# vocdoni/zk-franchise-proof-circuit

Measured on AMD Instinct MI355X. Metric: zkCensus proofs/sec (nLevels=160), higher is better.
Workload: dtype u256 (8 x u32 Montgomery, BN254 Fr/Fq)

## Files before the change

### include/zkcensus.h

```cpp
#ifndef ZKCENSUS_H
#define ZKCENSUS_H
#include <stddef.h>
#include <stdint.h>
#ifdef __cplusplus
extern "C" {
#endif

typedef struct zkc_ctx zkc_ctx;
typedef struct zkc_zkey zkc_zkey;

enum {
    ZKC_OK = 0,
    ZKC_ERR_GENERIC = 1,
    ZKC_ERR_SHORT_BUFFER = 2,
    ZKC_ERR_INVALID_WITNESS_LENGTH = 3,
    ZKC_ERR_BAD_ARG = 4,
    ZKC_ERR_FORMAT = 5,
    ZKC_ERR_HIP = 6,
    ZKC_ERR_WITNESS = 7
};
enum {
    ZKC_W_OK = 0, ZKC_W_ERR_WEIGHT = 1 , ZKC_W_ERR_SIK_ROOT = 2 ,
    ZKC_W_ERR_CENSUS_ROOT = 3 , ZKC_W_ERR_NULLIFIER = 4 , ZKC_W_ERR_LAST_SIBLING = 5 ,
    ZKC_W_ERR_INPUT_RANGE = 6 ,
// ... 64 lines not shown
                             uint8_t proof[256], uint8_t* publics, zkc_done_fn done, void* user);
int zkc_service_stats(zkc_service* svc, uint64_t out[8]);
int zkc_service_timing(zkc_service* svc, uint64_t out[8]);
int zkc_service_memory(zkc_service* svc, uint64_t out[8]);

int groth16_prover(const void* zkey_buffer, unsigned long zkey_size, const void* wtns_buffer, unsigned long wtns_size,
                   char* proof_buffer, unsigned long* proof_size, char* public_buffer, unsigned long* public_size,
                   char* error_msg, unsigned long error_msg_maxsize);

int groth16_fullprove(const void* zkey_buffer, unsigned long zkey_size, const void* wasm_buffer, unsigned long wasm_size, const char* inputs_json, unsigned long inputs_size,
                      char* proof_buffer, unsigned long* proof_size, char* public_buffer, unsigned long* public_size,
                      char* error_msg, unsigned long error_msg_maxsize);

int zkc_verify(const char* vkey_json, const char* public_json, const char* proof_json);
int zkc_verify_bin(const uint8_t* vk, int nPublic, const uint8_t* pub, const uint8_t* proof);

int zkc_pairing_bin(const uint8_t g1[64], const uint8_t g2[128], uint8_t out[384]);

int zkc_verify_batch(zkc_ctx* ctx, const uint8_t* vk, int nPublic, const uint8_t* pubs, const uint8_t* proofs, int N, const uint8_t* seed32);
const char* zkc_verify_last_error(void);

int zkc_proof_to_json(const uint8_t proof[256], const uint8_t* pub, int nPublic, char* proof_buf, unsigned long* proof_size,
                      char* public_buf, unsigned long* public_size);
int zkc_proof_from_json(const char* proof_json, const char* public_json, uint8_t proof[256], uint8_t* pub, int* nPublic);
int zkc_vkey_from_json(const char* vkey_json, uint8_t* vk, unsigned long* vk_size, int* nPublic);
int zkc_wtns_parse(const void* wtns_bytes, unsigned long size, const uint8_t** payload, uint32_t* nWitness);
unsigned long zkc_wtns_write(const void* payload, uint32_t nWitness, void* out, unsigned long out_size);

typedef struct zkc_msm zkc_msm;
int zkc_ntt_dev(zkc_ctx* ctx, const void* d_src, void* d_dst, int logn, int nvec, int inverse);
int zkc_g1_mul_batch_dev(zkc_ctx* ctx, const uint8_t base_std[64], const void* d_scalars, uint32_t n, void* d_out);
int zkc_msm_g1_load_dev(zkc_ctx* ctx, const void* d_bases_std, uint32_t n, zkc_msm** out);
int zkc_msm_g1_dev(zkc_msm* m, const void* d_scalars, uint8_t out[64]);
void zkc_msm_g1_free(zkc_msm* m);

int zkc_debug_stage(zkc_zkey* zk, const void* d_wtns, int stage, void* host_out);
unsigned long long zkc_debug_early_retries(void);
int zkc_msm_debug(zkc_zkey* zk, int which, const void* d_scalars, uint32_t count, void* host_out);
int zkc_debug_pairing_dev(zkc_ctx* ctx, const uint8_t* g1, const uint8_t* g2, const uint8_t* weights, int N, uint8_t product_out[384], uint8_t* folded_out,
                          int32_t* member_out, int* bad_out, const uint32_t* nodes, size_t count, uint8_t* node_out);

int zkc_poseidon_batch(zkc_ctx* ctx, int n_inputs, const void* inputs, size_t B, void* out);
int zkc_smt_build(zkc_ctx* ctx, const void* keys, const void* values, size_t n, int nLevels, uint8_t root[32], void* siblings, int32_t* depths);
int zkc_census_inputs(zkc_ctx* ctx, size_t n, int nLevels, const uint8_t election_id[64], const void* address, const void* password, const void* signature,
                      const void* available_weight, const void* vote_weight, const void* vote_hash, void* inputs_out, void* d_inputs_out, uint8_t* roots_out);

typedef struct zkc_tree zkc_tree;
enum {
    ZKC_TREE_OK = 0,
    ZKC_TREE_KEY_EXISTS = 1,
    ZKC_TREE_KEY_ABSENT = 2,
    ZKC_TREE_COLLISION = 3,
    ZKC_TREE_NOT_BELOW_R = 4,
    ZKC_TREE_NOT_IN_CENSUS = 5,
    ZKC_TREE_NOT_IN_SIK = 6,
    ZKC_TREE_SIK_MISMATCH = 7
};
int  zkc_tree_create(zkc_ctx* ctx, int nLevels, zkc_tree** out);
void zkc_tree_free(zkc_tree* tree);
int  zkc_tree_add(zkc_tree* tree, const void* keys, const void* values, size_t n, int32_t* status);
int  zkc_tree_update(zkc_tree* tree, const void* keys, const void* values, size_t n, int32_t* status);
int  zkc_tree_root(zkc_tree* tree, uint8_t root[32]);
int  zkc_tree_size(zkc_tree* tree, size_t* leaves);
int  zkc_tree_get(zkc_tree* tree, const void* keys, size_t n, void* values_out, int32_t* exists);
int  zkc_tree_gen_proof(zkc_tree* tree, const void* keys, size_t n, uint8_t root[32], void* siblings, int32_t* depths, int32_t* exists);
int  zkc_tree_census_inputs(zkc_tree* census, zkc_tree* sik, size_t n, const uint8_t election_id[64], const void* address, const void* password, const void* signature,
                            const void* vote_weight, const void* vote_hash, void* inputs_out, void* d_inputs_out, uint8_t roots_out[64], int32_t* status);
int  zkc_tree_stats(zkc_tree* tree, double ms[2]);

enum {
    ZKC_SMT_VALID = 0,
    ZKC_SMT_ROOT_MISMATCH = 1,
    ZKC_SMT_NOT_BELOW_R = 2,
    ZKC_SMT_LAST_SIBLING = 3,
    ZKC_SMT_KEY_PRESENT = 4,
    ZKC_SMT_OFF_PATH = 5
};
int zkc_smt_check_proofs(zkc_ctx* ctx, int nLevels, size_t n, const void* keys, const void* values, const void* siblings, const void* roots, int per_proof_roots,
                         int32_t* status);
int zkc_smt_check_stats(zkc_ctx* ctx, double ms[3]);

int zkc_profile_enable(zkc_ctx* ctx, uint32_t mask);
int zkc_profile_read(zkc_ctx* ctx, int category, double* total_ms, uint64_t* launches, uint64_t* alg_bytes);

int zkc_setup_from_r1cs(const char* r1cs_path, uint64_t seed, const char* zkey_path, const char* vkey_json_path,
                        char* err, size_t errlen);

#ifdef __cplusplus
}
#endif
#include "zkcensus_delete.h"
#include "zkcensus_snapshot.h"
#include "zkcensus_verify_each.h"
#include "zkcensus_setup.h"
#include "zkcensus_r1cs.h"
#include "zkcensus_phase2.h"
#endif
```

### zk-franchise-proof-circuit_amd/_native.py

```python
import ctypes
import os

_HERE = os.path.dirname(os.path.abspath(__file__))
LIB_PATH = os.environ.get('ZKCENSUS_LIB') or os.path.join(_HERE, 'libzkcensus.so')
_lib = None


class ZkcError(RuntimeError):
    def __init__(self, code, msg):
        super().__init__('libzkcensus error %d: %s' % (code, msg))
        self.code = code


def load():
    global _lib
    if _lib is not None:
        return _lib
    if not os.path.exists(LIB_PATH):
        raise ImportError('libzkcensus.so is not built (run `python -c "import __graft_entry__ as g; g.build()"`); '
                          'there is no CPU fallback for the product path')
    try:
        import torch
    except ImportError:
        pass
    L = ctypes.CDLL(LIB_PATH)
    vp, i32p = ctypes.c_void_p, ctypes.POINTER(ctypes.c_int32)
    L.zkc_ctx_create.argtypes = [ctypes.c_int, ctypes.POINTER(vp)]
    L.zkc_ctx_destroy.argtypes = [vp]
    L.zkc_last_error.argtypes = [vp]; L.zkc_last_error.restype = ctypes.c_char_p
    L.zkc_ctx_stream.argtypes = [vp]; L.zkc_ctx_stream.restype = vp
    L.zkc_witness.argtypes = [vp, ctypes.c_int, vp, ctypes.c_int, vp, i32p]
    L.zkc_witness_dev.argtypes = [vp, ctypes.c_int, vp, ctypes.c_int, vp, vp]
    u8p, u32p = ctypes.c_char_p, ctypes.POINTER(ctypes.c_uint32)
    L.zkc_zkey_load.argtypes = [vp, ctypes.c_char_p, ctypes.c_size_t, ctypes.POINTER(vp)]
    L.zkc_zkey_free.argtypes = [vp]; L.zkc_zkey_free.restype = None
    L.zkc_zkey_info.argtypes = [vp, u32p, u32p, u32p]
    L.zkc_zkey_pass_info.argtypes = [vp, ctypes.POINTER(ctypes.c_int), ctypes.POINTER(ctypes.c_int)]
    L.zkc_witness_status_text.argtypes = [ctypes.c_int, ctypes.c_int32]; L.zkc_witness_status_text.restype = ctypes.c_char_p
    L.zkc_prove.argtypes = [vp, ctypes.c_char_p, ctypes.c_uint32, u8p, u8p, ctypes.c_char_p, ctypes.c_char_p]
    L.zkc_prove_dev.argtypes = [vp, vp, ctypes.c_uint32, u8p, u8p, ctypes.c_char_p, ctypes.c_char_p]
    L.zkc_prove_batch_dev.argtypes = [vp, vp, ctypes.c_uint32, ctypes.c_int, ctypes.c_char_p, ctypes.c_char_p, ctypes.c_char_p]
    L.zkc_fullprove_batch_dev.argtypes = [vp, vp, ctypes.c_int, vp, vp, ctypes.c_char_p, ctypes.c_char_p, ctypes.c_char_p]
    L.zkc_debug_stage.argtypes = [vp, vp, ctypes.c_int, ctypes.c_char_p]
    L.zkc_debug_early_retries.argtypes = []; L.zkc_debug_early_retries.restype = ctypes.c_ulonglong
    L.zkc_msm_debug.argtypes = [vp, ctypes.c_int, vp, ctypes.c_uint32, ctypes.c_char_p]
    L.zkc_debug_pairing_dev.argtypes = [vp, ctypes.c_char_p, ctypes.c_char_p, ctypes.c_char_p, ctypes.c_int, ctypes.c_char_p, ctypes.c_char_p, i32p, ctypes.POINTER(ctypes.c_int),
                                        ctypes.POINTER(ctypes.c_uint32), ctypes.c_size_t, ctypes.c_char_p]
    ulp = ctypes.POINTER(ctypes.c_ulong)
    L.groth16_prover.argtypes = [ctypes.c_char_p, ctypes.c_ulong, ctypes.c_char_p, ctypes.c_ulong, ctypes.c_char_p, ulp, ctypes.c_char_p, ulp, ctypes.c_char_p, ctypes.c_ulong]
    L.zkc_verify.argtypes = [ctypes.c_char_p, ctypes.c_char_p, ctypes.c_char_p]
    L.zkc_verify_bin.argtypes = [ctypes.c_char_p, ctypes.c_int, ctypes.c_char_p, ctypes.c_char_p]
    L.zkc_verify_batch.argtypes = [vp, ctypes.c_char_p, ctypes.c_int, ctypes.c_char_p, ctypes.c_char_p, ctypes.c_int, ctypes.c_char_p]
    L.zkc_verify_batch_each.argtypes = [vp, ctypes.c_char_p, ctypes.c_int, ctypes.c_char_p, ctypes.c_char_p, ctypes.c_int, ctypes.c_char_p, i32p]
    L.zkc_verify_each_stats.argtypes = [vp, ctypes.POINTER(ctypes.c_uint64)]
    L.zkc_verify_last_error.restype = ctypes.c_char_p
    L.zkc_proof_to_json.argtypes = [ctypes.c_char_p, ctypes.c_char_p, ctypes.c_int, ctypes.c_char_p, ulp, ctypes.c_char_p, ulp]
    L.zkc_proof_from_json.argtypes = [ctypes.c_char_p, ctypes.c_char_p, ctypes.c_char_p, ctypes.c_char_p, ctypes.POINTER(ctypes.c_int)]
    L.zkc_vkey_from_json.argtypes = [ctypes.c_char_p, ctypes.c_char_p, ulp, ctypes.POINTER(ctypes.c_int)]
    L.zkc_wtns_parse.argtypes = [ctypes.c_char_p, ctypes.c_ulong, ctypes.POINTER(ctypes.c_void_p), ctypes.POINTER(ctypes.c_uint32)]
    L.zkc_wtns_write.argtypes = [ctypes.c_char_p, ctypes.c_uint32, ctypes.c_char_p, ctypes.c_ulong]; L.zkc_wtns_write.restype = ctypes.c_ulong
    L.zkc_poseidon_batch.argtypes = [vp, ctypes.c_int, ctypes.c_char_p, ctypes.c_size_t, ctypes.c_char_p]
    L.zkc_smt_build.argtypes = [vp, ctypes.c_char_p, ctypes.c_char_p, ctypes.c_size_t, ctypes.c_int, ctypes.c_char_p, ctypes.c_char_p, i32p]
    L.zkc_census_inputs.argtypes = [vp, ctypes.c_size_t, ctypes.c_int, ctypes.c_char_p, ctypes.c_char_p, ctypes.c_char_p, ctypes.c_char_p, ctypes.c_char_p, ctypes.c_char_p, ctypes.c_char_p, vp, vp, ctypes.c_char_p]
    sz = ctypes.c_size_t
    L.zkc_tree_create.argtypes = [vp, ctypes.c_int, ctypes.POINTER(vp)]
    L.zkc_tree_free.argtypes = [vp]; L.zkc_tree_free.restype = None
    L.zkc_tree_add.argtypes = [vp, ctypes.c_char_p, ctypes.c_char_p, sz, i32p]
    L.zkc_tree_update.argtypes = [vp, ctypes.c_char_p, ctypes.c_char_p, sz, i32p]
    L.zkc_tree_delete.argtypes = [vp, ctypes.c_char_p, sz, i32p]
    L.zkc_tree_refs.argtypes = [vp, ctypes.POINTER(sz)]
    L.zkc_tree_snapshot.argtypes = [vp, ctypes.POINTER(vp)]
    L.zkc_tree_snapshot_count.argtypes = [vp, ctypes.POINTER(sz)]
    L.zkc_tree_gen_absence_proof.argtypes = [vp, ctypes.c_char_p, sz, ctypes.c_char_p, vp, i32p, vp, vp, i32p, i32p]
    L.zkc_tree_root.argtypes = [vp, ctypes.c_char_p]
    L.zkc_tree_size.argtypes = [vp, ctypes.POINTER(sz)]
    L.zkc_tree_get.argtypes = [vp, ctypes.c_char_p, sz, vp, i32p]
    L.zkc_tree_gen_proof.argtypes = [vp, ctypes.c_char_p, sz, ctypes.c_char_p, vp, i32p, i32p]
    L.zkc_tree_census_inputs.argtypes = [vp, vp, sz, ctypes.c_char_p, ctypes.c_char_p, ctypes.c_char_p, ctypes.c_char_p, ctypes.c_char_p, ctypes.c_char_p, vp, vp, ctypes.c_char_p, i32p]
    L.zkc_tree_stats.argtypes = [vp, ctypes.POINTER(ctypes.c_double)]
    L.zkc_smt_check_proofs.argtypes = [vp, ctypes.c_int, sz, ctypes.c_char_p, ctypes.c_char_p, ctypes.c_char_p, ctypes.c_char_p, ctypes.c_int, i32p]
    L.zkc_smt_check_absence.argtypes = [vp, ctypes.c_int, sz, ctypes.c_char_p, ctypes.c_char_p, ctypes.c_char_p, i32p, ctypes.c_char_p, ctypes.c_char_p, ctypes.c_int, i32p]
    L.zkc_smt_check_stats.argtypes = [vp, ctypes.POINTER(ctypes.c_double)]
    L.zkc_profile_enable.argtypes = [vp, ctypes.c_uint32]
    L.zkc_ntt_dev.argtypes = [vp, vp, vp, ctypes.c_int, ctypes.c_int, ctypes.c_int]
    L.zkc_g1_mul_batch_dev.argtypes = [vp, ctypes.c_char_p, vp, ctypes.c_uint32, vp]
    L.zkc_msm_g1_load_dev.argtypes = [vp, vp, ctypes.c_uint32, ctypes.POINTER(vp)]
    L.zkc_msm_g1_dev.argtypes = [vp, vp, ctypes.c_char_p]
    L.zkc_msm_g1_free.argtypes = [vp]; L.zkc_msm_g1_free.restype = None
    L.zkc_profile_read.argtypes = [vp, ctypes.c_int, ctypes.POINTER(ctypes.c_double), ctypes.POINTER(ctypes.c_uint64), ctypes.POINTER(ctypes.c_uint64)]
    L.zkc_setup_from_r1cs.argtypes = [ctypes.c_char_p, ctypes.c_uint64, ctypes.c_char_p, ctypes.c_char_p, ctypes.c_char_p, ctypes.c_size_t]
    L.zkc_setup_from_r1cs_dev.argtypes = [vp, ctypes.c_char_p, ctypes.c_uint64, ctypes.c_char_p, ctypes.c_char_p, ctypes.c_char_p, ctypes.c_size_t]
    L.zkc_setup_stats.argtypes = [ctypes.POINTER(ctypes.c_double)]
    L.zkc_g1_fixed_mul_dev.argtypes = [vp, ctypes.c_char_p, vp, ctypes.c_uint32, vp]
    L.zkc_g2_fixed_mul_dev.argtypes = [vp, ctypes.c_char_p, vp, ctypes.c_uint32, vp]
    L.zkc_fixed_mul_window.argtypes = []
    L.zkc_circuit_nlevels_from_wasm.argtypes = [ctypes.c_char_p, ctypes.c_size_t, ctypes.c_char_p]
    L.zkc_sha256.argtypes = [ctypes.c_char_p, ctypes.c_size_t, ctypes.c_char_p]; L.zkc_sha256.restype = None
    L.zkc_zkey_sha256.argtypes = [vp, ctypes.c_char_p]
    L.zkc_zkey_fingerprint.argtypes = [ctypes.c_char_p, ctypes.c_size_t, ctypes.c_char_p]
    L.zkc_random_scalars.argtypes = [ctypes.c_char_p, ctypes.c_size_t]; L.zkc_random_scalars.restype = None
    L.zkc_pairing_bin.argtypes = [ctypes.c_char_p, ctypes.c_char_p, ctypes.c_char_p]
    L.zkc_pool_create.argtypes = [ctypes.POINTER(ctypes.c_int), ctypes.c_int, ctypes.POINTER(vp)]
    L.zkc_pool_destroy.argtypes = [vp]; L.zkc_pool_destroy.restype = None
    L.zkc_pool_size.argtypes = [vp]
    L.zkc_pool_ctx.argtypes = [vp, ctypes.c_int]; L.zkc_pool_ctx.restype = vp
    L.zkc_pool_zkey.argtypes = [vp, ctypes.c_int]; L.zkc_pool_zkey.restype = vp
    L.zkc_pool_last_error.argtypes = [vp]; L.zkc_pool_last_error.restype = ctypes.c_char_p
    L.zkc_pool_zkey_load.argtypes = [vp, ctypes.c_char_p, ctypes.c_size_t]
    L.zkc_pool_fullprove_batch.argtypes = [vp, ctypes.c_char_p, ctypes.c_int, ctypes.c_char_p, ctypes.c_char_p, ctypes.c_char_p, i32p]
    L.zkc_batch_begin.argtypes = [vp, ctypes.c_int, vp, ctypes.c_int, vp, vp, ctypes.c_char_p]
    L.zkc_batch_finish.argtypes = [vp, ctypes.c_int, ctypes.c_char_p, ctypes.c_char_p]
    L.zkc_service_create.argtypes = [ctypes.POINTER(ctypes.c_int), ctypes.c_int, ctypes.POINTER(vp)]
    L.zkc_service_destroy.argtypes = [vp]; L.zkc_service_destroy.restype = None
    L.zkc_service_default.argtypes = []; L.zkc_service_default.restype = vp
    L.zkc_service_last_error.restype = ctypes.c_char_p
    L.zkc_service_fullprove.argtypes = [vp, ctypes.c_char_p, ctypes.c_size_t, ctypes.c_int, ctypes.c_char_p, ctypes.c_char_p, ctypes.c_char_p, ctypes.c_char_p, i32p, ctypes.c_char_p, ctypes.c_size_t]
    L.zkc_service_prove.argtypes = [vp, ctypes.c_char_p, ctypes.c_size_t, ctypes.c_char_p, ctypes.c_uint32, ctypes.c_char_p, ctypes.c_char_p, ctypes.c_char_p, ctypes.c_char_p, ctypes.c_size_t]
    L.zkc_service_stats.argtypes = [vp, ctypes.POINTER(ctypes.c_uint64)]
    L.zkc_service_timing.argtypes = [vp, ctypes.POINTER(ctypes.c_uint64)]
    L.zkc_inputs_from_json.argtypes = [ctypes.c_char_p, ctypes.c_size_t, ctypes.c_int, ctypes.c_char_p, ctypes.c_char_p, ctypes.c_size_t]
    L.zkc_service_fullprove_json.argtypes = [vp, ctypes.c_char_p, ctypes.c_size_t, ctypes.c_char_p, ctypes.c_size_t, ctypes.c_char_p, ctypes.c_size_t, ctypes.c_char_p, ctypes.c_char_p, ctypes.c_char_p, i32p, ctypes.c_char_p, ctypes.c_size_t]
    L.groth16_fullprove.argtypes = [ctypes.c_char_p, ctypes.c_ulong, ctypes.c_char_p, ctypes.c_ulong, ctypes.c_char_p, ctypes.c_ulong, ctypes.c_char_p, ulp, ctypes.c_char_p, ulp, ctypes.c_char_p, ctypes.c_ulong]
    L.zkc_service_memory.argtypes = [vp, ctypes.POINTER(ctypes.c_uint64)]
    L.zkc_service_submit_fullprove.argtypes = [vp, ctypes.c_char_p, ctypes.c_size_t, ctypes.c_int, ctypes.c_char_p, ctypes.c_char_p, ctypes.c_char_p, ctypes.c_char_p, vp, vp]
    u32p_, i64p = u32p, ctypes.POINTER(ctypes.c_int64)
    L.zkc_r1cs_header_info.argtypes = [ctypes.c_char_p, sz, u32p_, u32p_, u32p_]
    L.zkc_r1cs_load.argtypes = [vp, ctypes.c_char_p, sz, ctypes.POINTER(vp)]
    L.zkc_r1cs_free.argtypes = [vp]; L.zkc_r1cs_free.restype = None
    L.zkc_r1cs_info.argtypes = [vp, u32p_, u32p_, u32p_]
    L.zkc_r1cs_check.argtypes = [vp, ctypes.c_char_p, ctypes.c_uint32, ctypes.c_int, i64p, u32p_]
    L.zkc_r1cs_check_dev.argtypes = [vp, vp, ctypes.c_uint32, ctypes.c_int, i64p, u32p_]
    L.zkc_r1cs_check_stats.argtypes = [vp, ctypes.POINTER(ctypes.c_double)]
    u64p = ctypes.POINTER(ctypes.c_uint64)
    szp = ctypes.POINTER(sz)
    L.zkc_g1_scale_dev.argtypes = [vp, vp, ctypes.c_uint32, ctypes.c_char_p, ctypes.c_int, vp]
    L.zkc_blake2b512.argtypes = [ctypes.c_char_p, sz, ctypes.c_char_p]; L.zkc_blake2b512.restype = None
    L.zkc_zkey_contributions.argtypes = [ctypes.c_char_p, sz, ctypes.c_char_p, u32p, ctypes.c_char_p, szp, ctypes.c_char_p, sz]
    L.zkc_zkey_contribute.argtypes = [vp, ctypes.c_char_p, sz, ctypes.c_char_p, ctypes.c_char_p, ctypes.c_char_p, szp, ctypes.c_char_p]
    L.zkc_zkey_verify_contributions.argtypes = [vp, ctypes.c_char_p, sz, ctypes.c_char_p, sz, ctypes.c_char_p, u32p, ctypes.c_char_p, sz]
    L.zkc_phase2_stats.argtypes = [ctypes.POINTER(ctypes.c_double)]
    L.zkc_debug_phase2_challenge_g2.argtypes = [ctypes.c_char_p, ctypes.c_char_p]
    L.zkc_debug_phase2_host_scale.argtypes = [ctypes.c_char_p, ctypes.c_uint32, ctypes.c_char_p, ctypes.c_int, ctypes.c_char_p, ctypes.POINTER(ctypes.c_double)]
    _lib = L
    return L


def declared_symbols(header='zkcensus.h'):
    import re
    hdr = open(os.path.join(_HERE, '..', 'include', header)).read()
    hdr = re.sub(r'/\*.*?\*/', '', hdr, flags=re.S)
    return sorted(set(re.findall(r'\b((?:zkc|groth16)_[a-z0-9_]+)\s*\(', hdr)))
```

### zk-franchise-proof-circuit_amd/csrc/zkc_api.hip

```cpp
#include "zkc_internal.h"
#include "zkc_f29.h"
#include "zkc_kernels.h"
#include <array>
#include <cstring>
#include <ctime>
#include <map>
#include <mutex>
#include "../../include/zkc_poseidon_constants.inc"

using namespace zkc;

static constexpr int ZKC_WITNESS_WAVE_MAX_B = 128, ZKC_WITNESS_WAVE_MAX_B_ALONE = 1024;

static thread_local std::string g_create_err;

int zkc_fail(zkc_ctx* ctx, int code, const std::string& msg) {
    if (ctx) ctx->err = msg; else g_create_err = msg;
    return code;
}
hipError_t zkc_wait_event(hipEvent_t ev, unsigned spin_us) {
    if (sw::on<sw::ZKC_SPIN_WAIT>()) return hipEventSynchronize(ev);
    timespec t0; if (spin_us) clock_gettime(CLOCK_MONOTONIC, &t0);
    for (int i = 0;; i++) {
        const hipError_t e = hipEventQuery(ev);
        if (e != hipErrorNotReady) return e;
        if (i < 48) continue;
        if (spin_us) { timespec t; clock_gettime(CLOCK_MONOTONIC, &t); if ((t.tv_sec - t0.tv_sec) * 1000000ll + (t.tv_nsec - t0.tv_nsec) / 1000 < (long long)spin_us) continue; spin_us = 0; }
        timespec ts{0, 50000}; nanosleep(&ts, nullptr);
    }
}
hipError_t zkc_wait_stream(hipStream_t st, hipEvent_t scratch_ev) {
    const hipError_t e = hipEventRecord(scratch_ev, st);
    return e != hipSuccess ? e : zkc_wait_event(scratch_ev);
}
int zkc_ensure(zkc_ctx* ctx, void** p, size_t* cur, size_t need) {
    if (*cur >= need) return ZKC_OK;
    if (*p) { ZKC_HIP_CHECK(ctx, hipFree(*p)); *p = nullptr; *cur = 0; }
    ZKC_HIP_CHECK(ctx, hipMalloc(p, need));
    *cur = need;
    return ZKC_OK;
}

void zkc_verify_ws_trim(zkc_ctx* ctx, size_t keep_bytes) {
    size_t total = 0; for (size_t b : ctx->vws_sz) total += b;
    if (total <= keep_bytes && keep_bytes) return;
    for (int i = 0; i < zkc_ctx::VWS_N; i++) { if (ctx->vws[i]) (void)hipFree(ctx->vws[i]); ctx->vws[i] = nullptr; ctx->vws_sz[i] = 0; }
}

static hipEvent_t prof_event(zkc_ctx* ctx) {
    if (!ctx->prof.free_events.empty()) { hipEvent_t e = ctx->prof.free_events.back(); ctx->prof.free_events.pop_back(); return e; }
    hipEvent_t e = nullptr; (void)hipEventCreate(&e); return e;
}
zkc_prof_scope::zkc_prof_scope(zkc_ctx* c, int category, uint64_t alg_bytes, hipStream_t stream) : ctx(c), cat(category), st(stream ? stream : (c ? c->stream : nullptr)) {
    on = c && ((c->prof.mask >> category) & 1u);
    if (!on) return;
    a = prof_event(c); b = prof_event(c);
    c->prof.bytes[cat] += alg_bytes; c->prof.launches[cat] += 1;
    (void)hipEventRecord(a, st);
}
zkc_prof_scope::~zkc_prof_scope() {
    if (!on) return;
    (void)hipEventRecord(b, st);
    ctx->prof.pending.push_back({a, b, cat});
}
extern "C" int zkc_profile_enable(zkc_ctx* ctx, uint32_t mask) {
    if (!ctx) return ZKC_ERR_BAD_ARG;
    ZKC_LOCK(ctx);
    ZKC_HIP_CHECK(ctx, hipSetDevice(ctx->device));
    (void)hipStreamSynchronize(ctx->stream);
    for (auto& r : ctx->prof.pending) { ctx->prof.free_events.push_back(r.a); ctx->prof.free_events.push_back(r.b); }
    ctx->prof.pending.clear();
    for (int i = 0; i < ZKC_PROF_NCAT; i++) { ctx->prof.ms[i] = 0; ctx->prof.launches[i] = 0; ctx->prof.bytes[i] = 0; }
    if (!ctx->d_prof_entries && hipMalloc((void**)&ctx->d_prof_entries, 8) != hipSuccess) ctx->d_prof_entries = nullptr;
    if (ctx->d_prof_entries) (void)hipMemset(ctx->d_prof_entries, 0, 8);
    ctx->prof.mask = mask;
    return ZKC_OK;
}
extern "C" int zkc_profile_read(zkc_ctx* ctx, int cat, double* total_ms, uint64_t* launches, uint64_t* alg_bytes) {
    if (!ctx || cat < 0 || cat >= ZKC_PROF_NCAT) return ZKC_ERR_BAD_ARG;
    ZKC_LOCK(ctx);
    ZKC_HIP_CHECK(ctx, hipSetDevice(ctx->device));
    ZKC_HIP_CHECK(ctx, hipStreamSynchronize(ctx->stream)); ZKC_HIP_CHECK(ctx, hipStreamSynchronize(ctx->stream2)); ZKC_HIP_CHECK(ctx, hipStreamSynchronize(ctx->fin_stream));
    for (auto& r : ctx->prof.pending) {
        float ms = 0; (void)hipEventElapsedTime(&ms, r.a, r.b); ctx->prof.ms[r.cat] += ms;
        ctx->prof.free_events.push_back(r.a); ctx->prof.free_events.push_back(r.b);
    }
    ctx->prof.pending.clear();
    if (cat == ZKC_PROF_MSM_G1_STREAMED && ctx->d_prof_entries) {
        unsigned long long v = 0; (void)hipMemcpyAsync(&v, ctx->d_prof_entries, 8, hipMemcpyDeviceToHost, ctx->stream); (void)hipStreamSynchronize(ctx->stream); ctx->prof.launches[cat] = v;
    }
    if (total_ms) *total_ms = ctx->prof.ms[cat]; if (launches) *launches = ctx->prof.launches[cat]; if (alg_bytes) *alg_bytes = ctx->prof.bytes[cat];
    return ZKC_OK;
}

extern "C" int zkc_poseidon_batch(zkc_ctx* ctx, int n_inputs, const void* inputs, size_t B, void* out) {
    if (!ctx || !inputs || !out || n_inputs < 2 || n_inputs > 4 || B == 0) return zkc_fail(ctx, ZKC_ERR_BAD_ARG, "zkc_poseidon_batch: bad argument");
    ZKC_LOCK(ctx);
    ZKC_HIP_CHECK(ctx, hipSetDevice(ctx->device));
    int rc;
    if ((rc = zkc_ensure(ctx, &ctx->d_scratch_in, &ctx->scratch_in_sz, B * n_inputs * 32))) return rc;
    if ((rc = zkc_ensure(ctx, &ctx->d_scratch_out, &ctx->scratch_out_sz, B * 32))) return rc;
    ZKC_HIP_CHECK(ctx, hipMemcpyAsync(ctx->d_scratch_in, inputs, B * n_inputs * 32, hipMemcpyHostToDevice, ctx->stream));
    hipLaunchKernelGGL(zkc_poseidon_batch_kernel, dim3((unsigned)((B + 63) / 64)), dim3(64), 0, ctx->stream, ctx->ptab, (const uint32_t*)ctx->d_scratch_in,
                       (uint32_t*)ctx->d_scratch_out, n_inputs, B);
    ZKC_HIP_CHECK(ctx, hipGetLastError());
    ZKC_HIP_CHECK(ctx, hipMemcpyAsync(out, ctx->d_scratch_out, B * 32, hipMemcpyDeviceToHost, ctx->stream));
    ZKC_HIP_CHECK(ctx, hipStreamSynchronize(ctx->stream));
    return ZKC_OK;
}

__global__ void zkc_status_combine(const int32_t* __restrict__ s3, int32_t* __restrict__ s, int B) {
    int b = blockIdx.x * blockDim.x + threadIdx.x;
    if (b >= B) return;
    int m = s3[3 * b + 2], c = s3[3 * b + 0], k = s3[3 * b + 1], r = 0;
    if (m == ZKC_W_ERR_INPUT_RANGE) r = m;
    else if (m == ZKC_W_ERR_WEIGHT) r = m;
    else if (k) r = k; else if (c) r = c; else r = m;
    s[b] = r;
}

template <size_t N>
static void conv_consts(std::vector<Fr>& out, const unsigned long long (&src)[N][4]) {
    for (size_t i = 0; i < N; i++) {
        uint32_t s[8];
        for (int k = 0; k < 4; k++) { s[2 * k] = (uint32_t)src[i][k]; s[2 * k + 1] = (uint32_t)(src[i][k] >> 32); }
        out.push_back(fp_from_std<FrParams>(s));
    }
}


extern "C" int zkc_ctx_create(int device, zkc_ctx** out) {
    if (!out) return zkc_fail(nullptr, ZKC_ERR_BAD_ARG, "out == NULL");
    int ndev = 0;
    if (hipGetDeviceCount(&ndev) != hipSuccess || ndev <= 0)
        return zkc_fail(nullptr, ZKC_ERR_HIP, "no HIP device: libzkcensus has no CPU path (the CPU restatement lives in oracle/ and is test-only)");
    if (device < 0 || device >= ndev) return zkc_fail(nullptr, ZKC_ERR_BAD_ARG, "bad device ordinal");
    zkc_ctx* ctx = new zkc_ctx();
    ctx->device = device;
    auto fail = [&](hipError_t e, const char* what) { g_create_err = std::string(what) + ": " + hipGetErrorString(e); delete ctx; return (int)ZKC_ERR_HIP; };
    hipError_t e;
    if ((e = hipSetDevice(device)) != hipSuccess) return fail(e, "hipSetDevice");
    { if (sw::on<sw::ZKC_DEVICE_BLOCKING_SYNC>() && hipSetDeviceFlags(hipDeviceScheduleBlockingSync) != hipSuccess) (void)hipGetLastError(); }
    if ((e = hipStreamCreateWithFlags(&ctx->stream, hipStreamNonBlocking)) != hipSuccess) return fail(e, "hipStreamCreate");
    if ((e = hipStreamCreateWithFlags(&ctx->stream2, hipStreamNonBlocking)) != hipSuccess) return fail(e, "hipStreamCreate(2)");
    if ((e = hipStreamCreateWithFlags(&ctx->fin_stream, hipStreamNonBlocking)) != hipSuccess) return fail(e, "hipStreamCreate(fin)");
    std::vector<Fr> all; size_t off[12]; int k = 0;
    off[k++] = all.size(); conv_consts(all, ZKC_POSEIDON_C3); off[k++] = all.size(); conv_consts(all, ZKC_POSEIDON_S3);
    off[k++] = all.size(); conv_consts(all, ZKC_POSEIDON_M3); off[k++] = all.size(); conv_consts(all, ZKC_POSEIDON_P3);
    off[k++] = all.size(); conv_consts(all, ZKC_POSEIDON_C4); off[k++] = all.size(); conv_consts(all, ZKC_POSEIDON_S4);
    off[k++] = all.size(); conv_consts(all, ZKC_POSEIDON_M4); off[k++] = all.size(); conv_consts(all, ZKC_POSEIDON_P4);
    off[k++] = all.size(); conv_consts(all, ZKC_POSEIDON_C5); off[k++] = all.size(); conv_consts(all, ZKC_POSEIDON_S5);
    off[k++] = all.size(); conv_consts(all, ZKC_POSEIDON_M5); off[k++] = all.size(); conv_consts(all, ZKC_POSEIDON_P5);
    if ((e = hipMalloc(&ctx->d_ptab_mem, all.size() * sizeof(Fr))) != hipSuccess) return fail(e, "hipMalloc(poseidon)");
    if ((e = hipMemcpy(ctx->d_ptab_mem, all.data(), all.size() * sizeof(Fr), hipMemcpyHostToDevice)) != hipSuccess) return fail(e, "hipMemcpy(poseidon)");
    const Fr* base = (const Fr*)ctx->d_ptab_mem;
    {
        std::vector<uint32_t> l29(all.size() * 12, 0);
        for (size_t i = 0; i < all.size(); i++) { uint32_t t9[9]; f29_from_fp_shl5(t9, all[i].v); f29_mul<FrParams>(&l29[12 * i], t9, F29K<FrParams>::one.l); }
        if ((e = hipMalloc(&ctx->d_ptab29_mem, l29.size() * 4)) != hipSuccess) return fail(e, "hipMalloc(poseidon29)");
        if ((e = hipMemcpy(ctx->d_ptab29_mem, l29.data(), l29.size() * 4, hipMemcpyHostToDevice)) != hipSuccess) return fail(e, "hipMemcpy(poseidon29)");
        ctx->ptab.base = base; ctx->ptab.base29 = (const uint32_t*)ctx->d_ptab29_mem;
        std::vector<uint32_t> k29; size_t koff[2];
        for (int t = 3; t <= 4; t++) {
            koff[t - 3] = k29.size();
            const int RP = t == 3 ? 57 : 56; const size_t oC = off[(t - 3) * 4 + 0], oS = off[(t - 3) * 4 + 1];
            for (int r = 0; r < RP; r++) for (int k = 0; k < t; k++) {
                const size_t si = oS + (size_t)(2 * t - 1) * r + (k ? t + k - 1 : 0), ci = oC + 5 * t + r;
                const Fr prod = all[si] * all[ci];
                uint32_t t9[9], o9[12] = {0}; f29_from_fp_shl5(t9, prod.v); f29_mul<FrParams>(o9, t9, F29K<FrParams>::one.l); f29_reduce_small<FrParams>(o9);
                k29.insert(k29.end(), o9, o9 + 12);
            }
        }
        if ((e = hipMalloc(&ctx->d_pk29_mem, k29.size() * 4)) != hipSuccess) return fail(e, "hipMalloc(poseidon K29)");
        if ((e = hipMemcpy(ctx->d_pk29_mem, k29.data(), k29.size() * 4, hipMemcpyHostToDevice)) != hipSuccess) return fail(e, "hipMemcpy(poseidon K29)");
// ... 135 lines not shown
```

### zk-franchise-proof-circuit_amd/csrc/zkc_internal.h

```cpp
#pragma once
#include <hip/hip_runtime.h>
#include <string>
#include <vector>
#include <map>
#include <mutex>
#include "../../include/zkcensus.h"
#include "zkc_device.h"
#include "zkc_switches.h"

#define ZKC_LOCK(ctx) std::lock_guard<std::recursive_mutex> _zkc_guard((ctx)->mu)
#define ZKC_HIP_CHECK(ctx, call)                                                                            \
    do { hipError_t _e = (call); if (_e != hipSuccess) {                                                     \
        return zkc_fail((ctx), ZKC_ERR_HIP, std::string(#call) + ": " + hipGetErrorString(_e)); } } while (0)

enum { ZKC_PROF_WITNESS = 0, ZKC_PROF_MATVEC = 1, ZKC_PROF_NTT = 2, ZKC_PROF_MSM_SORT = 3, ZKC_PROF_MSM_ACC_G1 = 4, ZKC_PROF_MSM_ACC_G2 = 5,
       ZKC_PROF_MSM_REDUCE = 6, ZKC_PROF_MSM_G1_STREAMED = 7 , ZKC_PROF_NCAT = 8 };
struct zkc_prof {
    uint32_t mask = 0;
    struct Rec { hipEvent_t a, b; int cat; };
    std::vector<Rec> pending; std::vector<hipEvent_t> free_events;
    double ms[ZKC_PROF_NCAT] = {0}; uint64_t launches[ZKC_PROF_NCAT] = {0}; uint64_t bytes[ZKC_PROF_NCAT] = {0};
};
struct zkc_ctx {
    std::recursive_mutex mu;
    int device = 0;
    hipStream_t stream = nullptr;
    hipStream_t stream2 = nullptr;
    hipStream_t fin_stream = nullptr;
    struct LaneStreams { hipStream_t st = nullptr, st2 = nullptr, fin = nullptr, red = nullptr; } lane_streams[4];
    struct zkc_lane* lanes = nullptr;
    hipEvent_t ev_acc_chain = nullptr; bool acc_chain_armed = false;
    std::string err;
    zkc::PoseidonTable ptab{};
    void* d_ptab_mem = nullptr;
    void* d_ptab29_mem = nullptr;
    void* d_pk29_mem = nullptr;
    std::map<int, uint32_t*> tmpl;
    struct TwiddleSet { uint32_t *fwd = nullptr, *inv = nullptr; void* ninv = nullptr; };
    std::map<int, TwiddleSet> ntt_tw;
    void* d_scratch_in = nullptr; size_t scratch_in_sz = 0;
    void* d_scratch_out = nullptr; size_t scratch_out_sz = 0;
    int32_t* d_status3 = nullptr; size_t status3_n = 0;
    int32_t* d_status = nullptr; size_t status_n = 0;
    enum { VWS_PTS = 0, VWS_RHO, VWS_IDX, VWS_GS, VWS_FOLD_TMP, VWS_FOLD_OUT, VWS_Q, VWS_LINES, VWS_TREE_A, VWS_TREE_B, VWS_BAD,
           VWS_FLAGS, VWS_SUM_TREE, VWS_TREE_ALL, VWS_NODES , VWS_N };
    void* vws[VWS_N] = {nullptr}; size_t vws_sz[VWS_N] = {0};
    uint64_t each_stats[4] = {0, 0, 0, 0};
    hipEvent_t ev_vws_up = nullptr, ev_vws_lines = nullptr;
    void* chk_h[2] = {nullptr, nullptr}; void* chk_d[2] = {nullptr, nullptr}; size_t chk_sz = 0; hipEvent_t chk_ev[2] = {nullptr, nullptr};
    double chk_ms[3] = {0, 0, 0};
    double r1cs_ms[3] = {0, 0, 0};
    zkc_prof prof;
    unsigned long long* d_prof_entries = nullptr;
};

int zkc_fail(zkc_ctx* ctx, int code, const std::string& msg);
hipError_t zkc_wait_event(hipEvent_t ev, unsigned spin_us = 0);
hipError_t zkc_wait_stream(hipStream_t st, hipEvent_t scratch_ev);
int zkc_ensure(zkc_ctx* ctx, void** p, size_t* cur, size_t need);
namespace zkc {
struct DevBuf {
    void* p = nullptr;
    DevBuf() = default;
    DevBuf(const DevBuf&) = delete;
    DevBuf& operator=(const DevBuf&) = delete;
    ~DevBuf() { if (p) (void)hipFree(p); }
    int alloc(zkc_ctx* ctx, size_t bytes) { ZKC_HIP_CHECK(ctx, hipMalloc(&p, bytes ? bytes : 4)); return ZKC_OK; }
    template <class T> T* as() const { return (T*)p; }
    void* release() { void* q = p; p = nullptr; return q; }
};
}
uint32_t* zkc_get_template(zkc_ctx* ctx, int nLevels);
int zkc_lane_streams(zkc_ctx* ctx, int l, bool with_red, zkc_ctx::LaneStreams* out);
int zkc_witness_chunk_async(zkc_ctx* ctx, int nLevels, const void* d_inputs, int B, void* d_wtns, int32_t* d_status3, int32_t* d_status, hipStream_t st);
void zkc_ctx_lanes_destroy(zkc_ctx* ctx);
inline int zkc_vws(zkc_ctx* ctx, int which, size_t need, void** out) { const int rc = zkc_ensure(ctx, &ctx->vws[which], &ctx->vws_sz[which], need); *out = ctx->vws[which]; return rc; }
void zkc_verify_ws_trim(zkc_ctx* ctx, size_t keep_bytes);
struct zkc_prof_scope {
    zkc_ctx* ctx; int cat; hipEvent_t a = nullptr, b = nullptr; bool on; hipStream_t st;
    zkc_prof_scope(zkc_ctx* c, int category, uint64_t alg_bytes, hipStream_t stream = nullptr);
    ~zkc_prof_scope();
};
```

### zk-franchise-proof-circuit_amd/csrc/zkc_msm.hip

```cpp
#include <cstdio>
#include <cstddef>
#include <ctime>
#include <cstdlib>
#include <cstring>
#include <string.h>
#include <vector>
#include "zkc_prover.h"
#include "zkc_f29.h"
#include "zkc_f29_g1.h"
#include "zkc_f29_g2.h"

namespace zkc {

template <class F> struct PointIO;
template <class PP> struct PointIO<Fp<PP>> {
    typedef Fp<PP> Fq;
    static __device__ __forceinline__ Affine<Fq> load(const Affine<Fq>* p) {
        const uint4* d = reinterpret_cast<const uint4*>(p); uint4 a = d[0], b = d[1], c = d[2], e = d[3];
        Affine<Fq> r;
        r.x.v[0] = a.x; r.x.v[1] = a.y; r.x.v[2] = a.z; r.x.v[3] = a.w; r.x.v[4] = b.x; r.x.v[5] = b.y; r.x.v[6] = b.z; r.x.v[7] = b.w;
        r.y.v[0] = c.x; r.y.v[1] = c.y; r.y.v[2] = c.z; r.y.v[3] = c.w; r.y.v[4] = e.x; r.y.v[5] = e.y; r.y.v[6] = e.z; r.y.v[7] = e.w;
        return r;
    }
};
// ... 301 lines not shown
    sh[threadIdx.x] = run; __syncthreads();
    for (int o = 1; o < 64; o <<= 1) {
        Acc29 v; f29_pt_set_inf(v);
        if ((int)threadIdx.x + o < 64) v = sh[threadIdx.x + o];
        __syncthreads();
        if ((int)threadIdx.x + o < 64) { Acc29 t = sh[threadIdx.x]; f29_pt_add(t, t, v); sh[threadIdx.x] = t; }
        __syncthreads();
    }
    if (threadIdx.x == 0) wres[2 * win.out + 1] = f29_pt_is_inf(sh[0]) ? XYZZ<Fq>::inf() : f29_pt_to_xyzz(sh[0]);
    Acc29 y; f29_pt_set_inf(y);
    if (threadIdx.x >= 1) { y = sh[threadIdx.x]; if (!f29_pt_is_inf(y)) for (int k = PER; k > 1; k >>= 1) f29_pt_dbl(y, y); }
    f29_pt_add(y, y, loc);
    __syncthreads();
    sh[threadIdx.x] = y; __syncthreads();
    for (int st = 32; st > 0; st >>= 1) {
        if ((int)threadIdx.x < st) { Acc29 t = sh[threadIdx.x]; f29_pt_add(t, t, sh[threadIdx.x + st]); sh[threadIdx.x] = t; }
        __syncthreads();
    }
    if (threadIdx.x == 0) wres[2 * win.out] = f29_pt_is_inf(sh[0]) ? XYZZ<Fq>::inf() : f29_pt_to_xyzz(sh[0]);
}
__global__ void __launch_bounds__(64)
zkc_msm_window29_g2(const XYZZ<Fq2>* __restrict__ partial, const uint32_t* __restrict__ segoff, const uint32_t* __restrict__ segcnt,
                    const MsmWindow* __restrict__ windows, XYZZ<Fq2>* __restrict__ wres, uint32_t max_segments) {
    __shared__ Acc29G2 sh[64];
    const MsmWindow win = windows[blockIdx.x];
    const int PER = (int)win.per;
    const uint32_t first = win.bucket0 + threadIdx.x * PER;
    Acc29G2 run, loc; f29g2_pt_set_inf(run); f29g2_pt_set_inf(loc);
    for (int k = PER - 1; k >= 0; k--) {
        uint32_t s0 = segoff[first + k], s1 = s0 + segcnt[first + k];
        if (s1 > max_segments) s1 = max_segments;
        for (uint32_t s = s0; s < s1; s++) { const XYZZ<Fq2> pq = partial[s]; if (!pq.is_inf()) { const Acc29G2 q = f29g2_pt_from_xyzz(pq); f29g2_pt_add(run, run, q); } }
        f29g2_pt_add(loc, loc, run);
    }
    sh[threadIdx.x] = run; __syncthreads();
    for (int o = 1; o < 64; o <<= 1) {
        Acc29G2 v; f29g2_pt_set_inf(v);
        if ((int)threadIdx.x + o < 64) v = sh[threadIdx.x + o];
        __syncthreads();
        if ((int)threadIdx.x + o < 64) { Acc29G2 t = sh[threadIdx.x]; f29g2_pt_add(t, t, v); sh[threadIdx.x] = t; }
        __syncthreads();
    }
    if (threadIdx.x == 0) wres[2 * win.out + 1] = f29g2_pt_is_inf(sh[0]) ? XYZZ<Fq2>::inf() : f29g2_pt_to_xyzz(sh[0]);
    Acc29G2 y; f29g2_pt_set_inf(y);
    if (threadIdx.x >= 1) { y = sh[threadIdx.x]; if (!f29g2_pt_is_inf(y)) for (int k = PER; k > 1; k >>= 1) f29g2_pt_dbl(y, y); }
    f29g2_pt_add(y, y, loc);
    __syncthreads();
    sh[threadIdx.x] = y; __syncthreads();
    for (int st = 32; st > 0; st >>= 1) {
        if ((int)threadIdx.x < st) { Acc29G2 t = sh[threadIdx.x]; f29g2_pt_add(t, t, sh[threadIdx.x + st]); sh[threadIdx.x] = t; }
        __syncthreads();
    }
    if (threadIdx.x == 0) wres[2 * win.out] = f29g2_pt_is_inf(sh[0]) ? XYZZ<Fq2>::inf() : f29g2_pt_to_xyzz(sh[0]);
}
__global__ void __launch_bounds__(MSM_MAX_VW_G1)
zkc_msm_final29(const XYZZ<Fq>* __restrict__ wres, const MsmJobList* __restrict__ jl, XYZZ<Fq>* __restrict__ results) {
    __shared__ Acc29 sh[MSM_MAX_VW_G1];
    const int j = blockIdx.x;
    const uint32_t vw = jl->job[j].vw, nvw = (1u << (jl->job[j].c - 1)) / vw, w0 = jl->job[j].win_off;
    int nt = 1; while ((uint32_t)nt < nvw) nt <<= 1;
    Acc29 Wk, Sk; f29_pt_set_inf(Wk); f29_pt_set_inf(Sk);
    if (threadIdx.x < nvw) {
        const XYZZ<Fq> a = wres[2 * (w0 + threadIdx.x)], b = wres[2 * (w0 + threadIdx.x) + 1];
        if (!a.is_inf()) Wk = f29_pt_from_xyzz(a);
        if (!b.is_inf()) Sk = f29_pt_from_xyzz(b);
    }
    sh[threadIdx.x] = Sk; __syncthreads();
    for (int o = 1; o < nt; o <<= 1) {
        Acc29 v; f29_pt_set_inf(v);
        if ((int)threadIdx.x + o < nt) v = sh[threadIdx.x + o];
        __syncthreads();
        if ((int)threadIdx.x + o < nt) { Acc29 t = sh[threadIdx.x]; f29_pt_add(t, t, v); sh[threadIdx.x] = t; }
        __syncthreads();
    }
    Acc29 y; f29_pt_set_inf(y);
    if (threadIdx.x >= 1 && (int)threadIdx.x < nt) { y = sh[threadIdx.x]; if (!f29_pt_is_inf(y)) for (uint32_t k = vw; k > 1; k >>= 1) f29_pt_dbl(y, y); }
    f29_pt_add(y, y, Wk);
    __syncthreads();
    sh[threadIdx.x] = y; __syncthreads();
    for (int st = nt / 2; st > 0; st >>= 1) {
        if ((int)threadIdx.x < st) { Acc29 t = sh[threadIdx.x]; f29_pt_add(t, t, sh[threadIdx.x + st]); sh[threadIdx.x] = t; }
        __syncthreads();
    }
    if (threadIdx.x == 0) results[j] = f29_pt_is_inf(sh[0]) ? XYZZ<Fq>::inf() : f29_pt_to_xyzz(sh[0]);
}

__global__ void __launch_bounds__(MSM_MAX_VW_PER_JOB)
zkc_msm_final29_g2(const XYZZ<Fq2>* __restrict__ wres, const MsmJobList* __restrict__ jl, XYZZ<Fq2>* __restrict__ results) {
    __shared__ Acc29G2 sh[MSM_MAX_VW_PER_JOB];
    const int j = blockIdx.x;
    const uint32_t vw = jl->job[j].vw, nvw = (1u << (jl->job[j].c - 1)) / vw, w0 = jl->job[j].win_off;
    int nt = 1; while ((uint32_t)nt < nvw) nt <<= 1;
    Acc29G2 Wk, Sk; f29g2_pt_set_inf(Wk); f29g2_pt_set_inf(Sk);
    if (threadIdx.x < nvw) {
        const XYZZ<Fq2> a = wres[2 * (w0 + threadIdx.x)], b = wres[2 * (w0 + threadIdx.x) + 1];
        if (!a.is_inf()) Wk = f29g2_pt_from_xyzz(a);
        if (!b.is_inf()) Sk = f29g2_pt_from_xyzz(b);
    }
    sh[threadIdx.x] = Sk; __syncthreads();
    for (int o = 1; o < nt; o <<= 1) {
        Acc29G2 v; f29g2_pt_set_inf(v);
        if ((int)threadIdx.x + o < nt) v = sh[threadIdx.x + o];
        __syncthreads();
        if ((int)threadIdx.x + o < nt) { Acc29G2 t = sh[threadIdx.x]; f29g2_pt_add(t, t, v); sh[threadIdx.x] = t; }
        __syncthreads();
    }
    Acc29G2 y; f29g2_pt_set_inf(y);
    if (threadIdx.x >= 1 && (int)threadIdx.x < nt) { y = sh[threadIdx.x]; if (!f29g2_pt_is_inf(y)) for (uint32_t k = vw; k > 1; k >>= 1) f29g2_pt_dbl(y, y); }
    f29g2_pt_add(y, y, Wk);
    __syncthreads();
    sh[threadIdx.x] = y; __syncthreads();
    for (int st = nt / 2; st > 0; st >>= 1) {
        if ((int)threadIdx.x < st) { Acc29G2 t = sh[threadIdx.x]; f29g2_pt_add(t, t, sh[threadIdx.x + st]); sh[threadIdx.x] = t; }
        __syncthreads();
    }
    if (threadIdx.x == 0) results[j] = f29g2_pt_is_inf(sh[0]) ? XYZZ<Fq2>::inf() : f29g2_pt_to_xyzz(sh[0]);
}

template <class F>
__global__ void __launch_bounds__(128)
zkc_msm_shift_bases(const Affine<F>* __restrict__ prev, Affine<F>* __restrict__ next, uint32_t count, int c) {
    const uint32_t i = blockIdx.x * blockDim.x + threadIdx.x;
    if (i >= count) return;
    Affine<F> a = PointIO<F>::load(prev + i);
    XYZZ<F> p = xyzz_dbl_affine(a);
    for (int k = 1; k < c; k++) p = xyzz_dbl(p);
    next[i] = xyzz_to_affine(p);
}
template <class F>
static int precompute(zkc_ctx* ctx, uint32_t count, Affine<F>* d_table, int c) {
    for (int w = 1; w < msm_nw(c); w++) {
        hipLaunchKernelGGL(HIP_KERNEL_NAME(zkc_msm_shift_bases<F>), dim3((count + 127) / 128), dim3(128), 0, ctx->stream,
                           d_table + (size_t)(w - 1) * count, d_table + (size_t)w * count, count, c);
        hipError_t e = hipGetLastError();
        if (e != hipSuccess) return zkc_fail(ctx, ZKC_ERR_HIP, std::string("zkc_msm_shift_bases: ") + hipGetErrorString(e));
    }
    return ZKC_OK;
}
int msm_precompute_g1(zkc_ctx* ctx, uint32_t count, G1Affine* d_table, int c) { return precompute<Fq>(ctx, count, d_table, c); }
int msm_precompute_g2(zkc_ctx* ctx, uint32_t count, G2Affine* d_table, int c) { return precompute<Fq2>(ctx, count, d_table, c); }
int msm_g2_rows29(zkc_ctx* ctx, const G2Affine* d_points, size_t n, const char* what, uint32_t** out) {
    DevBuf rows; int rc;
    if ((rc = rows.alloc(ctx, n * G2T29_WORDS * sizeof(uint32_t))) || (rc = msm_g2_table29(ctx, d_points, rows.as<uint32_t>(), n))) return rc;
    const hipError_t e = hipStreamSynchronize(ctx->stream);
    if (e != hipSuccess) return zkc_fail(ctx, ZKC_ERR_HIP, std::string(what) + ": " + hipGetErrorString(e));
    *out = (uint32_t*)rows.release();
    return ZKC_OK;
}
int msm_g2_window_table29(zkc_ctx* ctx, const G2Affine* d_bases, uint32_t count, int c, const char* what, uint32_t** out) {
    const size_t n = (size_t)msm_nw(c) * count;
    DevBuf shifted; int rc;
    if ((rc = shifted.alloc(ctx, n * sizeof(G2Affine)))) return rc;
    const hipError_t e = hipMemcpyAsync(shifted.p, d_bases, (size_t)count * sizeof(G2Affine), hipMemcpyDeviceToDevice, ctx->stream);
    if (e != hipSuccess) return zkc_fail(ctx, ZKC_ERR_HIP, std::string(what) + ": " + hipGetErrorString(e));
    if ((rc = msm_precompute_g2(ctx, count, shifted.as<G2Affine>(), c))) return rc;
    return msm_g2_rows29(ctx, shifted.as<G2Affine>(), n, what, out);
}

__device__ __forceinline__ uint32_t limb_of(const uint32_t k[8], int i) {
    uint32_t w = 0;
#pragma unroll
    for (int q = 0; q < 8; q++) w = (q == i) ? k[q] : w;
    return w;
}
template <class F>
__global__ void __launch_bounds__(64)
zkc_fold_mul(const Affine<F>* __restrict__ tbl, const uint32_t* __restrict__ scalars, const uint32_t* __restrict__ wires, uint32_t nw,
             int32_t pt_shift, XYZZ<F>* __restrict__ out) {
    const uint32_t i = blockIdx.x * blockDim.x + threadIdx.x;
    if (i >= nw) return;
    const uint32_t wire = wires[i];
    const uint4* sp = reinterpret_cast<const uint4*>(scalars + 8 * (size_t)wire); uint4 a = sp[0], b = sp[1];
    const uint32_t k[8] = {a.x, a.y, a.z, a.w, b.x, b.y, b.z, b.w};
    Affine<F> p = PointIO<F>::load(tbl + (uint32_t)((int32_t)wire - pt_shift));
    XYZZ<F> r = XYZZ<F>::inf();
    int top = -1;
#pragma unroll
    for (int q = 7; q >= 0; q--) if (top < 0 && k[q]) top = 32 * q + 31 - __clz(k[q]);
    for (int bit = top; bit >= 0; bit--) {
        r = xyzz_dbl(r);
        if ((limb_of(k, bit >> 5) >> (bit & 31)) & 1) r = xyzz_add_affine(r, p);
    }
    out[i] = r;
}
template <class F>
__global__ void __launch_bounds__(64)
zkc_fold_gsum(const XYZZ<F>* __restrict__ in, const uint32_t* __restrict__ gstart, uint32_t ngroups, XYZZ<F>* __restrict__ out) {
    const uint32_t g = blockIdx.x * blockDim.x + threadIdx.x;
    if (g >= ngroups) return;
    XYZZ<F> acc = XYZZ<F>::inf();
    for (uint32_t i = gstart[g], e = gstart[g + 1]; i < e; i++) acc = xyzz_add(acc, in[i]);
    out[g] = acc;
}
template <class F>
static int fold_group_sums(zkc_ctx* ctx, const Affine<F>* tbl, const uint32_t* d_scalars, const uint32_t* d_wires, uint32_t nw, int32_t pt_shift,
                           const uint32_t* d_gstart, uint32_t ngroups, XYZZ<F>* h_out) {
    DevBuf tmp, out; int rc;
    if ((rc = tmp.alloc(ctx, (size_t)nw * sizeof(XYZZ<F>))) || (rc = out.alloc(ctx, (size_t)ngroups * sizeof(XYZZ<F>)))) return rc;
    hipLaunchKernelGGL(HIP_KERNEL_NAME(zkc_fold_mul<F>), dim3((nw + 63) / 64), dim3(64), 0, ctx->stream, tbl, d_scalars, d_wires, nw, pt_shift, tmp.as<XYZZ<F>>());
// ... 213 lines not shown
```

### zk-franchise-proof-circuit_amd/csrc/zkc_msm_sort.hip

```cpp
#include "zkc_prover.h"
#include <algorithm>

namespace zkc {

struct TileState { uint32_t s[MSM_TILE_SCALARS / MSM_TILE][8]; uint32_t pt[MSM_TILE_SCALARS / MSM_TILE]; uint32_t carry[MSM_TILE_SCALARS / MSM_TILE]; bool live[MSM_TILE_SCALARS / MSM_TILE]; };
__device__ __forceinline__ void msm_tile_load(TileState& t, const MsmJob& job, uint32_t i0) {
#pragma unroll
    for (int k = 0; k < MSM_TILE_SCALARS / MSM_TILE; k++) {
        const uint32_t i = i0 + k * MSM_TILE;
        t.live[k] = i < job.count; t.pt[k] = 0; t.carry[k] = 0;
#pragma unroll
        for (int q = 0; q < 8; q++) t.s[k][q] = 0;
        if (t.live[k]) {
            const uint32_t wire = job.vmap ? job.vmap[i] : i;
            const uint4* sp = reinterpret_cast<const uint4*>(job.scalars + 8 * (size_t)wire); const uint4 a = sp[0], b = sp[1];
            t.s[k][0] = a.x; t.s[k][1] = a.y; t.s[k][2] = a.z; t.s[k][3] = a.w; t.s[k][4] = b.x; t.s[k][5] = b.y; t.s[k][6] = b.z; t.s[k][7] = b.w;
            t.pt[k] = (uint32_t)((int32_t)wire - job.pt_shift);
        }
    }
}
__device__ __forceinline__ uint32_t msm_tile_digit(TileState& t, int k, uint32_t w, uint32_t c, uint32_t& neg) {
    const uint32_t half = 1u << (c - 1), mask = (1u << c) - 1;
    const uint32_t bit = w * c, li = bit >> 5, sh = bit & 31;
    uint32_t lo = 0, hi = 0;
#pragma unroll
    for (int q = 0; q < 8; q++) { lo = ((uint32_t)q == li) ? t.s[k][q] : lo; hi = ((uint32_t)q == li + 1) ? t.s[k][q] : hi; }
    const uint64_t two = (uint64_t)lo | ((uint64_t)hi << 32);
    uint32_t d = (uint32_t)((two >> sh) & mask) + t.carry[k];
    neg = 0;
    if (d > half) { d = (1u << c) - d; neg = 1; t.carry[k] = 1; } else t.carry[k] = 0;
    return d;
}

__global__ void __launch_bounds__(MSM_TILE)
zkc_msm_count(const MsmJobList* __restrict__ jlp, const uint16_t* __restrict__ tilejob, uint32_t* __restrict__ tilecnt) {
    __shared__ uint32_t cnt[1u << MSM_MAX_HBITS];
    const MsmJobList& jl = *jlp;
    const uint32_t j = tilejob[blockIdx.x];
    const MsmJob job = jl.job[j];
    const uint32_t nbins = 1u << job.hbits, tile = blockIdx.x - job.tile0, ntiles = (job.count + MSM_TILE_SCALARS - 1) / MSM_TILE_SCALARS;
    for (uint32_t b = threadIdx.x; b < nbins; b += MSM_TILE) cnt[b] = 0;
    __syncthreads();
    TileState t; msm_tile_load(t, job, tile * MSM_TILE_SCALARS + threadIdx.x);
    for (uint32_t w = 0; w < job.nw; w++) {
#pragma unroll
        for (int k = 0; k < MSM_TILE_SCALARS / MSM_TILE; k++) { uint32_t neg; const uint32_t d = msm_tile_digit(t, k, w, job.c, neg); if (t.live[k] && d) atomicAdd(&cnt[(d - 1) >> job.lbits], 1u); }
    }
    __syncthreads();
    for (uint32_t b = threadIdx.x; b < nbins; b += MSM_TILE) tilecnt[job.cnt0 + b * ntiles + tile] = cnt[b];
}
__global__ void __launch_bounds__(256)
zkc_msm_binscan(const MsmJobList* __restrict__ jlp, uint32_t* __restrict__ tilecnt, uint32_t* __restrict__ hist, uint32_t* __restrict__ bin_start,
                unsigned long long* __restrict__ entry_counter) {
    __shared__ uint32_t part[256];
    __shared__ uint32_t carry_sh;
    const MsmJob& job = jlp->job[blockIdx.x];
    const uint32_t nbins = 1u << job.hbits, ntiles = (job.count + MSM_TILE_SCALARS - 1) / MSM_TILE_SCALARS, total = nbins * ntiles;
    uint32_t* c = tilecnt + job.cnt0;
    if (threadIdx.x == 0) carry_sh = job.ent_off;
    __syncthreads();
    for (uint32_t base = 0; base < total; base += 1024) {
        uint32_t v[4], sum = 0;
#pragma unroll
        for (int k = 0; k < 4; k++) { const uint32_t i = base + threadIdx.x * 4 + k; v[k] = i < total ? c[i] : 0; sum += v[k]; }
        part[threadIdx.x] = sum; __syncthreads();
        for (int o = 1; o < 256; o <<= 1) { uint32_t a = (int)threadIdx.x >= o ? part[threadIdx.x - o] : 0; __syncthreads(); part[threadIdx.x] += a; __syncthreads(); }
        uint32_t run = carry_sh + part[threadIdx.x] - sum;
#pragma unroll
        for (int k = 0; k < 4; k++) { const uint32_t i = base + threadIdx.x * 4 + k; if (i < total) c[i] = run; run += v[k]; }
        __syncthreads();
        if (threadIdx.x == 255) carry_sh = run;
        __syncthreads();
    }
    const uint32_t end = carry_sh;
    if (entry_counter && threadIdx.x == 0) atomicAdd(entry_counter, (unsigned long long)(end - job.ent_off));
    for (uint32_t b = threadIdx.x; b < nbins; b += 256) {
        const uint32_t st = c[b * ntiles], en = b + 1 < nbins ? c[(b + 1) * ntiles] : end;
        bin_start[job.bin0 + b] = st; hist[job.bin0 + b] = en - st;
    }
}
__global__ void __launch_bounds__(MSM_TILE)
zkc_msm_split(const MsmJobList* __restrict__ jlp, const uint16_t* __restrict__ tilejob, const uint32_t* __restrict__ tilecnt, uint32_t* __restrict__ vals) {
    __shared__ uint32_t cur[1u << MSM_MAX_HBITS];
    const MsmJobList& jl = *jlp;
    const uint32_t j = tilejob[blockIdx.x];
    const MsmJob job = jl.job[j];
    const uint32_t nbins = 1u << job.hbits, tile = blockIdx.x - job.tile0, ntiles = (job.count + MSM_TILE_SCALARS - 1) / MSM_TILE_SCALARS;
    for (uint32_t b = threadIdx.x; b < nbins; b += MSM_TILE) cur[b] = tilecnt[job.cnt0 + b * ntiles + tile];
    TileState t; msm_tile_load(t, job, tile * MSM_TILE_SCALARS + threadIdx.x);
    const uint32_t lowmask = (1u << job.lbits) - 1, lowshift = 31 - job.lbits;
    for (uint32_t w = 0; w < job.nw; w++) {
        __syncthreads();
#pragma unroll
        for (int k = 0; k < MSM_TILE_SCALARS / MSM_TILE; k++) {
            uint32_t neg; const uint32_t d = msm_tile_digit(t, k, w, job.c, neg);
            if (t.live[k] && d) {
                const uint32_t idx = d - 1, pos = atomicAdd(&cur[idx >> job.lbits], 1u);
                vals[pos] = (neg << 31) | ((idx & lowmask) << lowshift) | (t.pt[k] + w * job.tbl_count);
            }
        }
    }
}
template <bool CHUNKED>
__global__ void __launch_bounds__(256)
zkc_msm_bucket(const MsmJobList* __restrict__ jlp, const uint32_t* __restrict__ hist, const uint32_t* __restrict__ bin_start, const uint32_t* __restrict__ vals,
               uint32_t* __restrict__ vals2, uint32_t* __restrict__ off, uint32_t* __restrict__ bcnt) {
    __shared__ uint32_t cnt[256], pos[256];
    __shared__ uint32_t stage[256 * 32];
    const MsmJobList& jl = *jlp;
    const uint32_t bin = blockIdx.x, j = jl.job_of_bin(bin);
    const MsmJob& job = jl.job[j];
    const uint32_t lbits = job.lbits, nb2 = 1u << lbits, lowshift = 31 - lbits, lowmask = nb2 - 1, rowmask = (1u << lowshift) - 1;
    const uint32_t start = bin_start[bin], n = hist[bin];
    const uint32_t bucket_first = job.bucket0 + ((bin - job.bin0) << lbits);
    constexpr int BIG = 32, SMALL = 8;
    const bool in_regs = n <= 256u * BIG;
    uint32_t e[BIG];
    cnt[threadIdx.x] = 0; __syncthreads();
    if (in_regs) {
#pragma unroll
        for (int k = 0; k < BIG; k++) { const uint32_t i = k * 256 + threadIdx.x; e[k] = i < n ? vals[start + i] : 0u; }
#pragma unroll
        for (int k = 0; k < BIG; k++) if ((uint32_t)k * 256 + threadIdx.x < n) atomicAdd(&cnt[(e[k] >> lowshift) & lowmask], 1u);
    } else {
        for (uint32_t i0 = 0; i0 < n; i0 += 256 * SMALL) {
            uint32_t v[SMALL];
#pragma unroll
            for (int k = 0; k < SMALL; k++) { const uint32_t i = i0 + k * 256 + threadIdx.x; v[k] = i < n ? vals[start + i] : 0u; }
#pragma unroll
            for (int k = 0; k < SMALL; k++) if (i0 + k * 256 + threadIdx.x < n) atomicAdd(&cnt[(v[k] >> lowshift) & lowmask], 1u);
        }
    }
    __syncthreads();
    const uint32_t mine = cnt[threadIdx.x];
    pos[threadIdx.x] = mine; __syncthreads();
    for (int o = 1; o < 256; o <<= 1) { uint32_t a = (int)threadIdx.x >= o ? pos[threadIdx.x - o] : 0; __syncthreads(); pos[threadIdx.x] += a; __syncthreads(); }
    const uint32_t excl = pos[threadIdx.x] - mine;
    __syncthreads();
    if (threadIdx.x < nb2) { off[bucket_first + threadIdx.x] = start + excl; bcnt[bucket_first + threadIdx.x] = mine; }
    pos[threadIdx.x] = excl; __syncthreads();
    constexpr uint32_t excl_base = 0;
    if (in_regs) {
#pragma unroll
        for (int k = 0; k < BIG; k++) {
            if ((uint32_t)k * 256 < n) {
                if ((uint32_t)k * 256 + threadIdx.x < n) { const uint32_t p = atomicAdd(&pos[(e[k] >> lowshift) & lowmask], 1u) - excl_base; stage[p] = (e[k] & 0x80000000u) | (e[k] & rowmask); }
                __syncthreads();
            }
        }
        for (uint32_t i = threadIdx.x; i < n; i += 256) vals2[start + i] = stage[i];
    } else if constexpr (!CHUNKED) {
        for (uint32_t i0 = 0; i0 < n; i0 += 256 * SMALL) {
            uint32_t v[SMALL];
#pragma unroll
            for (int k = 0; k < SMALL; k++) { const uint32_t i = i0 + k * 256 + threadIdx.x; v[k] = i < n ? vals[start + i] : 0u; }
#pragma unroll
            for (int k = 0; k < SMALL; k++) {
                if (i0 + k * 256 + threadIdx.x < n) { const uint32_t p = atomicAdd(&pos[(v[k] >> lowshift) & lowmask], 1u); vals2[start + p] = (v[k] & 0x80000000u) | (v[k] & rowmask); }
// ... 190 lines not shown
```

### zk-franchise-proof-circuit_amd/csrc/zkc_prove.hip

```cpp
#include "zkc_prover.h"
#include "zkc_fixedbase.h"
#include "zkc_hostparse.h"
#include "zkc_host_util.h"
#include "zkc_kernels.h"
#include <cstring>
#include <ctime>
#include <cstdio>
#include <algorithm>
#include <atomic>

using namespace zkc;

static void matvec_launch(zkc_zkey* zk, zkc_lane& L, const uint32_t* d_wtns0, int nb, hipStream_t mv) {
    const uint32_t n = zk->n, nv = zk->nVars;
    const bool units = zk->n_unit_coeffs > 0 && nv <= 3 * (size_t)n && sw::on<sw::ZKC_MATVEC_UNITS>();
    if (units) hipLaunchKernelGGL(zkc_wtns_mont, dim3((nv + 255) / 256, nb), dim3(256), 0, mv, (const Fr*)d_wtns0, (size_t)nv, L.d_t, 3 * (size_t)n, nv);
    hipLaunchKernelGGL(zkc_matvec_jds, dim3((2 * n + 63 * zk->nlong + 255) / 256, nb), dim3(256), 0, mv, zk->d_perm, zk->d_rowlen, zk->d_jdptr, zk->d_col, zk->d_val,
                       (const Fr*)d_wtns0, (size_t)nv, L.d_abc, (int)n, zk->nlong, units ? (const Fr*)L.d_t : (const Fr*)nullptr, 3 * (size_t)n);
    hipLaunchKernelGGL(zkc_pointwise_mul, dim3((n + 255) / 256, nb), dim3(256), 0, mv, L.d_abc, (int)n);
}
static constexpr uint32_t MATVEC_LONG = 16;

namespace {
uint32_t rd32(const uint8_t* p) { uint32_t v; memcpy(&v, p, 4); return v; }
// ... 129 lines not shown
}
extern "C" int zkc_zkey_load(zkc_ctx* ctx, const void* zkey_bytes, size_t len, zkc_zkey** out) { return zkc::zkey_load_opts(ctx, zkey_bytes, len, 0, 0, out); }
size_t zkc::zkey_device_bytes(const zkc_zkey* zk, size_t* tables, size_t* work) {
    if (!zk) return 0;
    const size_t w = ctx_work_bytes(zk->ctx);
    if (tables) *tables = zk->bytes_tables; if (work) *work = w;
    return zk->bytes_tables + w;
}
int zkc::zkey_load_opts(zkc_ctx* ctx, const void* zkey_bytes, size_t len, int opt_lanes, int opt_inflight, zkc_zkey** out) {
    if (!ctx || !zkey_bytes || !out) return zkc_fail(ctx, ZKC_ERR_BAD_ARG, "zkc_zkey_load: bad argument");
    ZKC_LOCK(ctx);
    ZKC_HIP_CHECK(ctx, hipSetDevice(ctx->device));
    const size_t free_at_entry = dev_free_bytes(), work_at_entry = ctx_work_bytes(ctx);
    const uint8_t* buf = (const uint8_t*)zkey_bytes;
    parse::BinSections bs; parse::ZkeyHeader zh; std::string perr;
    if (!parse::binfile_sections(buf, len, "zkey", 1, bs, perr) || !parse::zkey_check(bs, zh, perr)) return zkc_fail(ctx, ZKC_ERR_FORMAT, perr);
    const uint8_t* const* sec = bs.sec;
    const uint8_t* h = sec[2];
    zkc_zkey* zk = new zkc_zkey(); zk->ctx = ctx;
    zk->nVars = zh.nVars; zk->nPub = zh.nPub; zk->n = zh.n; zk->logn = zh.logn; zk->nCoeffs = zh.nCoeffs;
    parse::sha256(buf, len, zk->sha256); parse::zkey_fingerprint(buf, len, bs, zk->fingerprint);
    const uint32_t n = zk->n, nv = zk->nVars, np = zk->nPub, nc = nv - np - 1;
    zk->alpha1 = rd_g1(h + 84); zk->beta1 = rd_g1(h + 148); zk->beta2 = rd_g2(h + 212); zk->gamma2 = rd_g2(h + 340);
    zk->delta1 = rd_g1(h + 468); zk->delta2 = rd_g2(h + 532);
    for (uint32_t i = 0; i <= np; i++) zk->ic.push_back(rd_g1(sec[3] + 64ull * i));
    {
        auto zero64 = [](const uint8_t* q) { for (int i = 0; i < 64; i++) if (q[i]) return false; return true; };
        zk->fold.infA.resize(nv); zk->fold.infB.resize(nv); zk->fold.infC.assign(nv, 0);
        for (uint32_t i = 0; i < nv; i++) { zk->fold.infA[i] = zero64(sec[5] + 64ull * i); zk->fold.infB[i] = zero64(sec[6] + 64ull * i); if (i > np) zk->fold.infC[i] = zero64(sec[8] + 64ull * (i - np - 1)); }
    }
    if (np == 8 && !sw::on<sw::ZKC_NO_FOLD>()) for (int nl = 3; nl <= 253; nl++) if ((uint32_t)WitnessLayout::make(nl).nWires == nv) { zk->nLevels = nl; break; }
    int rc = ZKC_OK;
    auto bail = [&](int code) { zkc_zkey_free(zk); return code; };
#define ZKC_HIP_BAIL(call)                                                                                      \
    do { hipError_t _e = (call); if (_e != hipSuccess) return bail(zkc_fail(ctx, ZKC_ERR_HIP, std::string(#call) + ": " + hipGetErrorString(_e))); } while (0)
#define ZKC_UP(dst, src, bytes) ZKC_HIP_BAIL(hipMemcpy((dst), (src), (bytes), hipMemcpyHostToDevice))
    {
        std::vector<uint32_t> rowptr(2 * (size_t)n + 1, 0), col(zk->nCoeffs); std::vector<Fr> val(zk->nCoeffs);
        const uint8_t* c = sec[4] + 4;
        for (uint32_t i = 0; i < zk->nCoeffs; i++) {
            uint32_t m = rd32(c + 44ull * i), cc = rd32(c + 44ull * i + 4), s = rd32(c + 44ull * i + 8);
            rowptr[(size_t)m * n + cc + 1]++;
        }
        for (size_t r = 0; r < 2 * (size_t)n; r++) rowptr[r + 1] += rowptr[r];
        std::vector<uint32_t> fill(rowptr.begin(), rowptr.end() - 1);
        for (uint32_t i = 0; i < zk->nCoeffs; i++) {
            uint32_t m = rd32(c + 44ull * i), cc = rd32(c + 44ull * i + 4), s = rd32(c + 44ull * i + 8);
            uint32_t k = fill[(size_t)m * n + cc]++;
            col[k] = s; memcpy(val[k].v, c + 44ull * i + 12, 32);
        }
        const size_t nrows = 2 * (size_t)n;
        const JdsLayout J = jds_layout(nrows, [&](uint32_t r) { return rowptr[r + 1] - rowptr[r]; }, MATVEC_LONG);
        const std::vector<uint32_t>&perm = J.perm, &rowlen = J.rowlen, &jdptr = J.jdptr;
        zk->nlong = J.nlong;
        std::vector<uint32_t> jcol(zk->nCoeffs); std::vector<Fr> jval(zk->nCoeffs);
        if (nv >= (1u << 30)) return bail(zkc_fail(ctx, ZKC_ERR_FORMAT, "zkey too large for 30-bit wire indices"));
        Fr one_r2, neg_r2; for (int i = 0; i < 8; i++) one_r2.v[i] = FrParams::r2[i];
        neg_r2 = Fr::zero() - one_r2;
        zk->n_unit_coeffs = (uint32_t)jds_fill(J, [&](uint32_t r, uint32_t k) { const size_t src = (size_t)rowptr[r] + k; return std::pair<uint32_t, Fr>(col[src], val[src]); },
                                               one_r2, neg_r2, jcol.data(), jval.data());
        if ((rc = dmalloc(ctx, &zk->d_perm, nrows)) || (rc = dmalloc(ctx, &zk->d_rowlen, nrows)) || (rc = dmalloc(ctx, &zk->d_jdptr, jdptr.size())) ||
            (rc = dmalloc(ctx, &zk->d_col, jcol.size() + 1)) || (rc = dmalloc(ctx, &zk->d_val, jval.size() + 1))) return bail(rc);
        ZKC_UP(zk->d_perm, perm.data(), nrows * 4); ZKC_UP(zk->d_rowlen, rowlen.data(), nrows * 4); ZKC_UP(zk->d_jdptr, jdptr.data(), jdptr.size() * 4);
        ZKC_UP(zk->d_col, jcol.data(), jcol.size() * 4);
        ZKC_UP(zk->d_val, jval.data(), jval.size() * sizeof(Fr));
    }
    {
        TwiddleTables tw;
        if ((rc = ntt_twiddle_tables(ctx, (int)zk->logn, true, &tw))) return bail(rc);
        zk->d_tw_fwd = tw.fwd; zk->d_tw_inv = tw.inv; zk->d_tw_fwd29 = tw.fwd29; zk->d_tw_inv29 = tw.inv29;
        const Fr g = fr_root_of_unity((int)zk->logn + 1), ninv = fp_inv<FrParams>(fp_from_u32<FrParams>(n));
        std::vector<Fr> cs(n);
        cs[0] = ninv; for (uint32_t i = 1; i < n; i++) cs[i] = cs[i - 1] * g;
        if ((rc = dmalloc(ctx, &zk->d_coset, n))) return bail(rc);
        ZKC_UP(zk->d_coset, cs.data(), cs.size() * sizeof(Fr));
        if ((rc = ntt_bitrev_table(ctx, zk->d_coset, &zk->d_coset_br, (int)zk->logn))) return bail(rc);
    }
    { const auto e_c = sw::given<sw::ZKC_C_SECTIONS>(); zk->c_sec = e_c ? (int)*e_c : zk->nLevels >= 0 ? MSM_C_SMALL : msm_c_for(nv); }
    { const auto e_h = sw::given<sw::ZKC_C_H>(); zk->c_h = e_h ? (int)*e_h : zk->nLevels >= 0 ? MSM_C_BIG : std::max(msm_c_for(n), n >= 12000 ? 15 : 12); }
    const int NWS = msm_nw(zk->c_sec);
    { const int dt = (int)sw::value<sw::ZKC_DEEP_TABLES>(1); const auto e_c = sw::given<sw::ZKC_C_DEEP>();
      const int cd = e_c ? (int)*e_c : msm_c_for(dt == 2 ? (size_t)40000 : (size_t)nv * 4 / 5);
      zk->c_deep = (zk->nLevels >= 0 && (nv >= (1u << 16) || dt == 2) && zk->c_sec < cd && dt != 0) ? cd : 0; }
    zk->c_h = std::max(zk->c_h, std::max(zk->c_sec, zk->c_deep));
    const int NWB = msm_nw(zk->c_h);
    zk->offA = 0; zk->offB1 = NWS * nv; zk->offC = 2 * NWS * nv; zk->offH = 2 * NWS * nv + NWS * nc;
    const int NWD = zk->c_deep ? msm_nw(zk->c_deep) : 0;
    zk->offA_deep = zk->offH + NWB * n; zk->offB1_deep = zk->offA_deep + NWD * nv; zk->offC_deep = zk->offB1_deep + NWD * nv;
    const size_t g1_points = (size_t)NWS * (2 * (size_t)nv + nc) + (size_t)NWB * n + (size_t)NWD * (2 * (size_t)nv + nc);
    if (g1_points >= (1ull << 31)) return bail(zkc_fail(ctx, ZKC_ERR_FORMAT, "zkey too large for 31-bit point indices"));
    if ((rc = dmalloc(ctx, &zk->d_g1, g1_points)) || (rc = dmalloc(ctx, &zk->d_g2, (size_t)NWS * nv))) return bail(rc);
    ZKC_UP(zk->d_g1 + zk->offA, sec[5], 64ull * nv); ZKC_UP(zk->d_g1 + zk->offB1, sec[6], 64ull * nv);
    ZKC_UP(zk->d_g1 + zk->offC, sec[8], 64ull * nc); ZKC_UP(zk->d_g1 + zk->offH, sec[9], 64ull * n);
    ZKC_UP(zk->d_g2, sec[7], 128ull * nv);
    if ((rc = msm_precompute_g1(ctx, nv, zk->d_g1 + zk->offA, zk->c_sec)) || (rc = msm_precompute_g1(ctx, nv, zk->d_g1 + zk->offB1, zk->c_sec)) ||
        (rc = msm_precompute_g1(ctx, nc, zk->d_g1 + zk->offC, zk->c_sec)) || (rc = msm_precompute_g1(ctx, n, zk->d_g1 + zk->offH, zk->c_h)) ||
        (rc = msm_precompute_g2(ctx, nv, zk->d_g2, zk->c_sec))) return bail(rc);
    if ((rc = dmalloc(ctx, &zk->d_g2_29, 60 * (size_t)NWS * nv)) || (rc = msm_g2_table29(ctx, zk->d_g2, zk->d_g2_29, (size_t)NWS * nv))) return bail(rc);
    if (zk->c_deep) {
        ZKC_UP(zk->d_g1 + zk->offA_deep, sec[5], 64ull * nv); ZKC_UP(zk->d_g1 + zk->offB1_deep, sec[6], 64ull * nv); ZKC_UP(zk->d_g1 + zk->offC_deep, sec[8], 64ull * nc);
        if ((rc = msm_precompute_g1(ctx, nv, zk->d_g1 + zk->offA_deep, zk->c_deep)) || (rc = msm_precompute_g1(ctx, nv, zk->d_g1 + zk->offB1_deep, zk->c_deep)) ||
            (rc = msm_precompute_g1(ctx, nc, zk->d_g1 + zk->offC_deep, zk->c_deep))) return bail(rc);
        if ((rc = msm_g2_window_table29(ctx, zk->d_g2, nv, zk->c_deep, "second section tables", &zk->d_g2_29_deep))) return bail(rc);
    }
    {
        if (sw::on<sw::ZKC_G2_LONE_TABLE>() && (zk->nLevels >= 0 || nv < (1u << 16))) {
            if ((rc = msm_g2_window_table29(ctx, zk->d_g2, nv, MSM_C_G2_LONE, "lone-proof G2 table", &zk->d_g2_29_lone))) return bail(rc);
        }
    }
    const auto e_inf = sw::given<sw::ZKC_INFLIGHT>();
    zk->max_inflight = opt_inflight > 0 ? std::min(opt_inflight, MSM_MAX_JOBS / 4) : e_inf ? (int)*e_inf : zk->nLevels >= 0 ? 64 : 96;
    {
        const size_t per_proof_entries = (size_t)NWS * 3 * nv + (size_t)NWB * n, census_pass = 96ull * (22ull * 3 * 82754 + 15ull * 131072);
        const int fit = (int)std::max<size_t>(1, census_pass / std::max<size_t>(per_proof_entries, 1));
        zk->max_inflight = std::min(zk->max_inflight, fit);
    }
    { const auto e_l = sw::given<sw::ZKC_LANES>(); zk->nlanes = opt_lanes > 0 ? std::min(opt_lanes, (int)MAX_LANES) : e_l ? (int)*e_l : zk->nLevels >= 0 ? (int)MAX_LANES : 1; }
    zk->serial_streams = sw::on<sw::ZKC_SERIAL_STREAMS>();
    if ((rc = lanes_ensure(zk, 1, 0, 1))) return bail(rc);
    {
        FixedBase<Fq> td(zk->delta1), ta(zk->alpha1), tb(zk->beta1); FixedBase<Fq2> t2(zk->delta2);
        if ((rc = dmalloc(ctx, &zk->d_tblDelta1, td.tab.size())) || (rc = dmalloc(ctx, &zk->d_tblAlpha1, ta.tab.size())) ||
            (rc = dmalloc(ctx, &zk->d_tblBeta1, tb.tab.size())) || (rc = dmalloc(ctx, &zk->d_tblDelta2, t2.tab.size()))) return bail(rc);
        ZKC_UP(zk->d_tblDelta1, td.tab.data(), td.tab.size() * sizeof(G1Affine)); ZKC_UP(zk->d_tblAlpha1, ta.tab.data(), ta.tab.size() * sizeof(G1Affine));
        ZKC_UP(zk->d_tblBeta1, tb.tab.data(), tb.tab.size() * sizeof(G1Affine)); ZKC_UP(zk->d_tblDelta2, t2.tab.data(), t2.tab.size() * sizeof(G2Affine));
    }
    ZKC_HIP_BAIL(hipStreamSynchronize(ctx->stream));
    if (zk->nLevels >= 0 && (rc = fold_prepare(zk))) return bail(rc);
    if ((rc = fb4_prepare(zk))) return bail(rc);
    { const size_t f = dev_free_bytes(), grown = ctx_work_bytes(ctx) > work_at_entry ? ctx_work_bytes(ctx) - work_at_entry : 0; zk->bytes_tables = free_at_entry > f + grown ? free_at_entry - f - grown : 0; }
    *out = zk;
    return ZKC_OK;
#undef ZKC_UP
#undef ZKC_HIP_BAIL
}

int zkc::prove_reserve(zkc_zkey* zk, int inflight) {
    if (!zk) return ZKC_ERR_BAD_ARG;
    ZKC_LOCK(zk->ctx);
    ZKC_HIP_CHECK(zk->ctx, hipSetDevice(zk->ctx->device));
    return lanes_ensure(zk, inflight);
}
extern "C" int zkc_zkey_pass_info(const zkc_zkey* zk, int* pass_size, int* lanes) {
    if (!zk) return ZKC_ERR_BAD_ARG;
    if (pass_size) *pass_size = zk->max_inflight; if (lanes) *lanes = zk->nlanes;
    return ZKC_OK;
}
extern "C" int zkc_zkey_info(const zkc_zkey* zk, uint32_t* nVars, uint32_t* nPublic, uint32_t* domainSize) {
    if (!zk) return ZKC_ERR_BAD_ARG;
    if (nVars) *nVars = zk->nVars; if (nPublic) *nPublic = zk->nPub; if (domainSize) *domainSize = zk->n;
    return ZKC_OK;
}

static std::vector<std::pair<int, int>> fold_group_ranges(const WitnessLayout& L, int tree) {
    std::vector<std::pair<int, int>> r; const int n = L.n, blk = tree == 0 ? L.off_census : L.off_sikver;
    for (int g = 0; g < n - 1; g++) {
        const int nctrl = (g == n - 3) + (g > 0 && g < n - 2) + 1;
        r.push_back({blk + L.lvl_off(g) + nctrl, blk + (g + 1 < n - 1 ? L.lvl_off(g + 1) : L.lvl_off(n - 1))});
    }
    r.push_back({blk + L.off_n2bold, blk + L.off_n2bold + 253 + 127 + 133});
    return r;
}
template <class X> static void suffix_sums(std::vector<X>& suf, const X* g, int n) {
    suf.assign(n, X::inf());
    for (int D = n - 2; D >= 0; D--) suf[D] = xyzz_add(suf[D + 1], g[D]);
}
template <class PT> static int fold_upload(zkc_ctx* ctx, PT** d, const std::vector<PT>& b, const std::vector<PT>* suf) {
    std::vector<PT> t; t.push_back(b[0]); t.insert(t.end(), suf[0].begin(), suf[0].end()); t.insert(t.end(), suf[1].begin(), suf[1].end());
    ZKC_HIP_CHECK(ctx, hipMalloc((void**)d, t.size() * sizeof(PT)));
    ZKC_HIP_CHECK(ctx, hipMemcpy(*d, t.data(), t.size() * sizeof(PT), hipMemcpyHostToDevice));
    return ZKC_OK;
}
static int fold_prepare(zkc_zkey* zk) {
    if (zk->fold.ready) return ZKC_OK;
    zkc_ctx* ctx = zk->ctx; const WitnessLayout L = WitnessLayout::make(zk->nLevels); const int n = L.n;
    uint32_t* tmpl = zkc_get_template(ctx, zk->nLevels); if (!tmpl) return ZKC_ERR_HIP;
    std::vector<uint32_t> wires, gstart;
    for (int tree = 0; tree < 2; tree++) for (auto& rg : fold_group_ranges(L, tree)) { gstart.push_back((uint32_t)wires.size()); for (int w = rg.first; w < rg.second; w++) wires.push_back((uint32_t)w); }
    gstart.push_back((uint32_t)wires.size());
// ... 46 lines not shown
    return ZKC_OK;
}
static int fold_vmap(zkc_zkey* zk, int Dc, int Ds, zkc_zkey::Fold::VMap* out) {
    auto it = zk->fold.vmaps.find({Dc, Ds});
    if (it != zk->fold.vmaps.end()) { *out = it->second; return ZKC_OK; }
    zkc_ctx* ctx = zk->ctx; const WitnessLayout L = WitnessLayout::make(zk->nLevels); const int n = L.n;
    std::vector<uint8_t> folded(L.nWires, 0);
    for (int tree = 0; tree < 2; tree++) {
        auto rg = fold_group_ranges(L, tree); const int D = tree == 0 ? Dc : Ds;
        for (int g = D; g < n - 1; g++) for (int w = rg[g].first; w < rg[g].second; w++) folded[w] = 1;
        for (int w = rg[n - 1].first; w < rg[n - 1].second; w++) folded[w] = 1;
    }
    std::vector<uint32_t> v; zkc_zkey::Fold::VMap m;
    m.offA = 0; for (int w = 0; w < L.nWires; w++) if (!folded[w] && !zk->fold.infA[w]) v.push_back((uint32_t)w); m.nA = (uint32_t)v.size();
    m.offB = (uint32_t)v.size(); for (int w = 0; w < L.nWires; w++) if (!folded[w] && !zk->fold.infB[w]) v.push_back((uint32_t)w); m.nB = (uint32_t)v.size() - m.offB;
    m.offC = (uint32_t)v.size(); for (int w = (int)zk->nPub + 1; w < L.nWires; w++) if (!folded[w] && !zk->fold.infC[w]) v.push_back((uint32_t)w); m.nC = (uint32_t)v.size() - m.offC;
    ZKC_HIP_CHECK(ctx, hipMalloc((void**)&m.d, v.size() * 4 + 4));
    ZKC_HIP_CHECK(ctx, hipMemcpyAsync(m.d, v.data(), v.size() * 4, hipMemcpyHostToDevice, ctx->stream));
    ZKC_HIP_CHECK(ctx, hipStreamSynchronize(ctx->stream));
    zk->fold.vmaps[{Dc, Ds}] = m; *out = m;
    return ZKC_OK;
}

static int nofold_vmap(zkc_zkey* zk, zkc_zkey::Fold::VMap* out) {
    auto it = zk->fold.vmaps.find({-1, -1});
    if (it != zk->fold.vmaps.end()) { *out = it->second; return ZKC_OK; }
    zkc_ctx* ctx = zk->ctx; const uint32_t nv = zk->nVars, np = zk->nPub;
    std::vector<uint32_t> v; zkc_zkey::Fold::VMap m;
    m.offA = 0; for (uint32_t w = 0; w < nv; w++) if (!zk->fold.infA[w]) v.push_back(w); m.nA = (uint32_t)v.size();
    m.offB = (uint32_t)v.size(); for (uint32_t w = 0; w < nv; w++) if (!zk->fold.infB[w]) v.push_back(w); m.nB = (uint32_t)v.size() - m.offB;
    m.offC = (uint32_t)v.size(); for (uint32_t w = np + 1; w < nv; w++) if (!zk->fold.infC[w]) v.push_back(w); m.nC = (uint32_t)v.size() - m.offC;
    if ((size_t)m.nA + m.nB + m.nC + (size_t)nv / 50 < 3 * (size_t)nv - np - 1) {
        ZKC_HIP_CHECK(ctx, hipMalloc((void**)&m.d, v.size() * 4 + 4));
        ZKC_HIP_CHECK(ctx, hipMemcpyAsync(m.d, v.data(), v.size() * 4, hipMemcpyHostToDevice, ctx->stream));
        ZKC_HIP_CHECK(ctx, hipStreamSynchronize(ctx->stream));
    }
    zk->fold.vmaps[{-1, -1}] = m; *out = m;
    return ZKC_OK;
}

static int h_matvec_dev(zkc_zkey* zk, zkc_lane& L, const uint32_t* d_wtns0, int nb, hipStream_t mv) {
    zkc_ctx* ctx = zk->ctx; const uint32_t n = zk->n, nv = zk->nVars;
    zkc_prof_scope _ps(ctx, ZKC_PROF_MATVEC, (uint64_t)nb * ((uint64_t)zk->nCoeffs * 68 + 3ull * n * 32), mv);
    matvec_launch(zk, L, d_wtns0, nb, mv);
    ZKC_HIP_CHECK(ctx, hipGetLastError());
    return ZKC_OK;
}
static int h_evals_dev(zkc_zkey* zk, zkc_lane& L, hipStream_t st, const uint32_t* d_wtns0, int nb, bool with_matvec = true) {
    zkc_ctx* ctx = zk->ctx; const uint32_t n = zk->n;
    if (with_matvec) { int rc0 = h_matvec_dev(zk, L, d_wtns0, nb, st); if (rc0) return rc0; }
    zkc_prof_scope _pn(ctx, ZKC_PROF_NTT, (uint64_t)nb * (6ull * 2 * n * 32 + 4ull * n * 32), st);
    int rc;
    if (!sw::on<sw::ZKC_NTT_SEPARATE>() && zk->logn >= 12 && zk->logn <= 27) {
        if ((rc = ntt_pair_run(ctx, st, L.d_abc, zk->d_tw_inv29, zk->d_tw_fwd29, zk->d_coset_br, (int)zk->logn, 3 * nb))) return rc;
    } else {
        if ((rc = ntt_run(ctx, st, L.d_abc, L.d_t, zk->d_tw_inv29, zk->d_coset, (int)zk->logn, 3 * nb))) return rc;
        if ((rc = ntt_run(ctx, st, L.d_t, L.d_abc, zk->d_tw_fwd29, nullptr, (int)zk->logn, 3 * nb))) return rc;
    }
    hipLaunchKernelGGL(zkc_join_abc, dim3((n + 255) / 256, nb), dim3(256), 0, st, L.d_abc, L.d_p, (int)n);
    ZKC_HIP_CHECK(ctx, hipGetLastError());
    return ZKC_OK;
}

extern "C" int zkc_debug_stage(zkc_zkey* zk, const void* d_wtns, int stage, void* host_out) {
    if (!zk || !d_wtns || !host_out) return ZKC_ERR_BAD_ARG;
    zkc_ctx* ctx = zk->ctx; const uint32_t n = zk->n;
    ZKC_LOCK(ctx);
    ZKC_HIP_CHECK(ctx, hipSetDevice(ctx->device)); ZKC_HIP_CHECK(ctx, hipStreamSynchronize(ctx->stream));
    { int rc0 = lanes_ensure(zk, 1, 0, 1); if (rc0) return rc0; }
    zkc_lane& L0 = ctx->lanes[0]; const hipStream_t st0 = lane_st(zk, L0).st;
    if (stage == 0) {
        matvec_launch(zk, L0, (const uint32_t*)d_wtns, 1, st0);
        ZKC_HIP_CHECK(ctx, hipGetLastError());
        ZKC_HIP_CHECK(ctx, hipMemcpyAsync(host_out, L0.d_abc, 96ull * n, hipMemcpyDeviceToHost, st0));
    } else {
        int rc = h_evals_dev(zk, L0, st0, (const uint32_t*)d_wtns, 1); if (rc) return rc;
        ZKC_HIP_CHECK(ctx, hipMemcpyAsync(host_out, L0.d_p, 32ull * n, hipMemcpyDeviceToHost, st0));
    }
    ZKC_HIP_CHECK(ctx, hipStreamSynchronize(st0));
    return ZKC_OK;
}

extern "C" int zkc_msm_debug(zkc_zkey* zk, int which, const void* d_scalars, uint32_t count, void* host_out) {
    if (!zk || !d_scalars || !host_out || which < 0 || which > 4) return ZKC_ERR_BAD_ARG;
    zkc_ctx* ctx = zk->ctx;
    ZKC_LOCK(ctx);
    ZKC_HIP_CHECK(ctx, hipSetDevice(ctx->device)); ZKC_HIP_CHECK(ctx, hipStreamSynchronize(ctx->stream));
    { int rc0 = lanes_ensure(zk, 1, 0, 1); if (rc0) return rc0; }
    zkc_lane& L0 = ctx->lanes[0]; const hipStream_t st_l0 = lane_st(zk, L0).st;
    const uint32_t full = which == 3 ? zk->nVars - zk->nPub - 1 : which == 4 ? zk->n : zk->nVars;
    if (count != full) return zkc_fail(ctx, ZKC_ERR_BAD_ARG, "zkc_msm_debug: count must equal the section size");
    static thread_local MsmJobList jl; jl.clear(256, 1024, which == 2 ? (uint32_t)MSM_MAX_VW_PER_JOB : (uint32_t)MSM_MAX_VW_G1);
    const uint32_t offs[5] = {zk->offA, zk->offB1, 0, zk->offC, zk->offH};
    jl.add((const uint32_t*)d_scalars, nullptr, count, offs[which], full, 0, which == 4 ? zk->c_h : zk->c_sec);
    int rc = which == 2 ? msm_pass_g2(zk, L0.w2, jl, 0, true, st_l0) : msm_pass_g1(zk, L0.w1, jl, 0, true, st_l0); if (rc) return rc;
    ZKC_HIP_CHECK(ctx, hipStreamSynchronize(st_l0));
    if (which == 2) wr_g2_std((uint8_t*)host_out, xyzz_to_affine(*(G2XYZZ*)L0.w2.h_results));
    else wr_g1_std((uint8_t*)host_out, xyzz_to_affine(*(G1XYZZ*)L0.w1.h_results));
    return ZKC_OK;
}

int zkc::prove_batch_begin(zkc_zkey* zk, int cs, const void* d_wtns, uint32_t nWitness, int B, const uint8_t* rs, bool want_publics, const void* d_inputs, int32_t* d_status,
                           int lane0, hipEvent_t wait_first, const uint8_t* host_depths, bool no_early) {
    if (!zk || !d_wtns || !rs || B <= 0 || cs < 0 || cs >= CALL_SLOTS || lane0 >= zk->nlanes) return zkc_fail(zk ? zk->ctx : nullptr, ZKC_ERR_BAD_ARG, "zkc_prove_batch_dev: bad argument");
    zkc_ctx* ctx = zk->ctx;
    ZKC_LOCK(ctx);
    if (nWitness != zk->nVars) return zkc_fail(ctx, ZKC_ERR_INVALID_WITNESS_LENGTH, "Invalid witness length. Circuit: " + std::to_string(zk->nVars) + ", witness: " + std::to_string(nWitness));
    for (int b = 0; b < 2 * B; b++) { uint32_t t[8]; memcpy(t, rs + 32 * (size_t)b, 32); if (!fp_std_lt_p<FrParams>(t)) return zkc_fail(ctx, ZKC_ERR_BAD_ARG, "r or s >= field order"); }
    ZKC_HIP_CHECK(ctx, hipSetDevice(ctx->device));
    const uint32_t nv = zk->nVars, np = zk->nPub, nc = nv - np - 1, n = zk->n;
    const bool can_fold = zk->nLevels >= 0;
    WitnessLayout L{}; int rc;
    {
        const int npasses0 = (B + zk->max_inflight - 1) / zk->max_inflight, per0 = (B + npasses0 - 1) / npasses0;
        if ((rc = lanes_ensure(zk, per0, lane0 >= 0 ? lane0 : 0, lane0 >= 0 ? 1 : std::min(zk->nlanes, npasses0)))) return rc;
    }
    hipStream_t st0 = (lane0 >= 0 && !zk->serial_streams && B <= zk->max_inflight) ? ctx->lanes[lane0].st : ctx->stream;
    zkc_zkey::CallSlot& CS = zk->call[cs];
    if (CS.pending) return zkc_fail(ctx, ZKC_ERR_BAD_ARG, "prove_batch_begin: this call slot has a call in flight (finish it first)");
    if (CS.cap < (size_t)B) {
        if (CS.d_rs) { ZKC_HIP_CHECK(ctx, hipFree(CS.d_rs)); ZKC_HIP_CHECK(ctx, hipFree(CS.d_proofs)); ZKC_HIP_CHECK(ctx, hipHostFree(CS.h_out)); ZKC_HIP_CHECK(ctx, hipHostFree(CS.h_rs)); ZKC_HIP_CHECK(ctx, hipFree(CS.d_xyzz)); ZKC_HIP_CHECK(ctx, hipHostFree(CS.h_xyzz));
                       CS.d_rs = CS.d_proofs = CS.h_out = CS.h_rs = CS.d_xyzz = CS.h_xyzz = nullptr; CS.cap = 0; }
        const size_t want = std::max<size_t>((size_t)B, std::max<size_t>(256, std::min<size_t>(2 * CS.cap, 4096)));
        ZKC_HIP_CHECK(ctx, hipMalloc((void**)&CS.d_rs, 64 * want)); ZKC_HIP_CHECK(ctx, hipMalloc((void**)&CS.d_proofs, 256 * want));
        ZKC_HIP_CHECK(ctx, hipHostMalloc((void**)&CS.h_out, (256 + 32 * (size_t)zk->nPub) * want)); ZKC_HIP_CHECK(ctx, hipHostMalloc((void**)&CS.h_rs, 64 * want));
        ZKC_HIP_CHECK(ctx, hipMalloc((void**)&CS.d_xyzz, 512 * want)); ZKC_HIP_CHECK(ctx, hipHostMalloc((void**)&CS.h_xyzz, 512 * want)); CS.cap = want;
    }
    static const unsigned ev_host_flags = hipEventDisableTiming;
    for (int l = 0; l < zk->nlanes; l++) if (!CS.ev_done[l]) ZKC_HIP_CHECK(ctx, hipEventCreateWithFlags(&CS.ev_done[l], ev_host_flags));
    CS.as_xyzz.assign((size_t)B, 0); CS.lanes_used = 0;
    if (wait_first) ZKC_HIP_CHECK(ctx, hipStreamWaitEvent(st0, wait_first, 0));
    uint8_t* const h_pub = CS.h_out + 256ull * CS.cap;
    if (rs != CS.h_rs_copy.data()) CS.h_rs_copy.assign(rs, rs + 64 * (size_t)B);
    memcpy(CS.h_rs, rs, 64 * (size_t)B);
    ZKC_HIP_CHECK(ctx, hipMemcpyAsync(CS.d_rs, CS.h_rs, 64 * (size_t)B, hipMemcpyHostToDevice, st0));
    uint32_t* tmpl = nullptr;
    if (can_fold) {
        L = WitnessLayout::make(zk->nLevels);
        if ((rc = fold_prepare(zk))) return rc;
        tmpl = zkc_get_template(ctx, zk->nLevels); if (!tmpl) return ZKC_ERR_HIP;
        const size_t nflags = (size_t)B * 2 * L.n;
        if (CS.flags_cap < nflags) {
            if (CS.d_flags) { ZKC_HIP_CHECK(ctx, hipFree(CS.d_flags)); ZKC_HIP_CHECK(ctx, hipHostFree(CS.h_flags)); CS.d_flags = CS.h_flags = nullptr; CS.flags_cap = 0; }
            const size_t want = std::max(nflags, (size_t)256 * 2 * L.n);
            ZKC_HIP_CHECK(ctx, hipMalloc((void**)&CS.d_flags, want * 4)); ZKC_HIP_CHECK(ctx, hipHostMalloc((void**)&CS.h_flags, want * 4)); CS.flags_cap = want;
        }
    }
    CS.early_n = 0; CS.arg_wtns = d_wtns; CS.arg_nw = nWitness; CS.arg_publics = want_publics; CS.arg_lane0 = lane0; CS.arg_inputs = d_inputs != nullptr; CS.arg_wait = nullptr;
    const size_t ecap = MSM_MAX_JOBS / 4;
    const bool early_wanted = !no_early && can_fold && B <= zk->max_inflight && (B <= 2 ? zk->d_fb4 != nullptr : sw::on<sw::ZKC_EARLY_LAYOUT>());
    if (early_wanted && !CS.h_early) { ZKC_HIP_CHECK(ctx, hipHostMalloc((void**)&CS.h_early, (ecap + ecap * 2 * 256) * 4)); CS.early_cap = ecap; }
    if (early_wanted && host_depths) {
        bool ok = true; for (int i = 0; i < 2 * B; i++) ok = ok && host_depths[i] < (uint8_t)L.n && L.n <= 255;
        if (ok) { CS.early_n = B; CS.early_depth.assign(host_depths, host_depths + 2 * (size_t)B); }
    } else if (early_wanted && d_inputs) {
        if (!zk->d_depths) { ZKC_HIP_CHECK(ctx, hipMalloc((void**)&zk->d_depths, 2 * ecap * 4)); ZKC_HIP_CHECK(ctx, hipHostMalloc((void**)&zk->h_depths, 2 * ecap * 4)); }
        uint32_t* hd = zk->h_depths;
        if (wait_first) ZKC_HIP_CHECK(ctx, hipStreamWaitEvent(ctx->stream2, wait_first, 0));
        hipLaunchKernelGGL(zkc_input_depths, dim3(B, 2), dim3(64), 0, ctx->stream2, (const uint32_t*)d_inputs, L.nInputs, L.n, zk->d_depths);
        ZKC_HIP_CHECK(ctx, hipGetLastError());
        ZKC_HIP_CHECK(ctx, hipMemcpyAsync(hd, zk->d_depths, 8 * (size_t)B, hipMemcpyDeviceToHost, ctx->stream2));
        ZKC_HIP_CHECK(ctx, hipStreamSynchronize(ctx->stream2));
        bool ok = true; for (int i = 0; i < 2 * B; i++) ok = ok && hd[i] < (uint32_t)L.n;
        if (ok) { CS.early_n = B; CS.early_depth.resize(2 * (size_t)B); for (int i = 0; i < 2 * B; i++) CS.early_depth[i] = (uint8_t)hd[i]; }
    }
    const int npasses = (B + zk->max_inflight - 1) / zk->max_inflight;
    const int per_pass = (B + npasses - 1) / npasses;
    while ((int)CS.ev_chunk.size() < npasses) { hipEvent_t e; ZKC_HIP_CHECK(ctx, hipEventCreateWithFlags(&e, ev_host_flags)); CS.ev_chunk.push_back(e); }
    int32_t* d_status3 = nullptr;
    if (d_inputs) {
        if ((rc = zkc_ensure(ctx, (void**)&CS.d_status3, &CS.status3_cap, std::max<size_t>((size_t)B, 256) * 3 * sizeof(int32_t)))) return rc;
        d_status3 = CS.d_status3;
    }
    const int wgroup = (int)sw::value<sw::ZKC_WITNESS_GROUP>(8);
    for (int c = 0; c < npasses; c++) {
        const int p0 = c * per_pass, nb = std::min(per_pass, B - p0);
        uint32_t* wc = (uint32_t*)d_wtns + (size_t)p0 * nv * 8;
        if (d_inputs && (c % wgroup == 0 || c == 1)) {
            const int glast = c == 0 ? 1 : std::min(((c / wgroup) + 1) * wgroup, npasses);
            const int g0 = p0, gn = std::min((glast - c) * per_pass, B - g0);
            if (gn > 0 && (rc = zkc_witness_chunk_async(ctx, zk->nLevels, (const uint8_t*)d_inputs + (size_t)g0 * L.nInputs * 32, gn, wc, d_status3 + 3 * (size_t)g0, d_status + g0, st0))) return rc;
        }
        if (can_fold) {
            uint32_t* fl = CS.d_flags + (size_t)p0 * 2 * L.n;
            hipLaunchKernelGGL(zkc_fold_check, dim3(L.n, 2, nb), dim3(64), 0, st0, L, (const uint32_t*)wc, tmpl, fl, nb);
            ZKC_HIP_CHECK(ctx, hipGetLastError());
            ZKC_HIP_CHECK(ctx, hipMemcpyAsync(CS.h_flags + (size_t)p0 * 2 * L.n, fl, (size_t)nb * 2 * L.n * 4, hipMemcpyDeviceToHost, st0));
        }
        if (CS.early_n) {
            if (d_status) ZKC_HIP_CHECK(ctx, hipMemcpyAsync(CS.h_early, d_status, 4 * (size_t)B, hipMemcpyDeviceToHost, st0));
            else memset(CS.h_early, 0, 4 * (size_t)B);
            ZKC_HIP_CHECK(ctx, hipMemcpyAsync(CS.h_early + CS.early_cap, CS.d_flags + (size_t)p0 * 2 * L.n, (size_t)nb * 2 * L.n * 4, hipMemcpyDeviceToHost, st0));
        }
        ZKC_HIP_CHECK(ctx, hipEventRecord(CS.ev_chunk[c], st0));
    }
    const bool trace_host = sw::on<sw::ZKC_TRACE_HOST>();
    auto now_ms = [] { timespec t; clock_gettime(CLOCK_MONOTONIC, &t); return t.tv_sec * 1e3 + t.tv_nsec * 1e-6; };
    const double t_begin = now_ms(); double tr[6] = {0};
    int pass = 0, done_on_st_lane = -1;
    const bool one_lane = lane0 >= 0 || zk->nlanes == 1;
    for (int p0 = 0; p0 < B; p0 += per_pass, pass++) {
        const int nb = std::min(per_pass, B - p0);
        const int li = lane0 >= 0 ? lane0 : pass % zk->nlanes; CS.lanes_used |= 1u << li;
        zkc_lane& LN = ctx->lanes[li]; const LaneSt LS = lane_st(zk, LN); const int slot = LN.npass & 1;
        tr[0] = now_ms();
        const bool early = CS.early_n > 0;
        if (!early) ZKC_HIP_CHECK(ctx, zkc_wait_event(CS.ev_chunk[pass]));
        tr[1] = now_ms();
        ZKC_HIP_CHECK(ctx, hipStreamWaitEvent(LS.st, CS.ev_chunk[pass], 0)); ZKC_HIP_CHECK(ctx, hipStreamWaitEvent(LS.st2, CS.ev_chunk[pass], 0));
        hipStream_t st = LS.st, st2 = LS.st2, fin = LS.fin;
        const uint32_t* w0 = (const uint32_t*)d_wtns + (size_t)p0 * nv * 8;
        uint8_t dcq[MSM_MAX_JOBS / 4], dsq[MSM_MAX_JOBS / 4]; bool fold = can_fold;
        if (early) for (int q = 0; q < nb; q++) { dcq[q] = CS.early_depth[2 * q]; dsq[q] = CS.early_depth[2 * q + 1]; }
        else for (int q = 0; q < nb && fold; q++) for (int t = 0; t < 2; t++) {
            const uint32_t* f = CS.h_flags + ((size_t)(p0 + q) * 2 + t) * L.n;
            if (f[L.n - 1]) { fold = false; break; }
            int D = 0; for (int g = 0; g < L.n - 1; g++) if (f[g]) D = g + 1;
            (t == 0 ? dcq : dsq)[q] = (uint8_t)D;
        }
        static thread_local zkc_zkey::Fold::VMap vms[MSM_MAX_JOBS / 4];
        if (fold) for (int q = 0; q < nb; q++) if ((rc = fold_vmap(zk, dcq[q], dsq[q], &vms[q]))) return rc;
        const bool nofold_lists = sw::on<sw::ZKC_NOFOLD_LISTS>();
        if (!fold && nofold_lists) {
            zkc_zkey::Fold::VMap nf; if ((rc = nofold_vmap(zk, &nf))) return rc;
            for (int q = 0; q < nb; q++) vms[q] = nf;
        }
        const bool listed = fold || (nofold_lists && vms[0].d != nullptr);
        if (LN.npass >= 2) { ZKC_HIP_CHECK(ctx, hipStreamWaitEvent(st, LN.ev_fin[slot], 0)); ZKC_HIP_CHECK(ctx, hipStreamWaitEvent(st2, LN.ev_fin[slot], 0)); }
        LN.npass++;
        const bool mv_prefetch = !sw::on<sw::ZKC_MATVEC_INLINE>() && one_lane;
        const bool mv_done = mv_prefetch && pass > 0;
        if (mv_done) ZKC_HIP_CHECK(ctx, hipStreamWaitEvent(st, LN.ev_mv, 0));
        if ((rc = h_evals_dev(zk, LN, st, w0, nb, !mv_done))) return rc;
        ZKC_HIP_CHECK(ctx, hipEventRecord(LN.ev_ntt, st));
        tr[2] = now_ms();
        static thread_local MsmJobList j1, j2;
        const uint32_t vwb_env = (uint32_t)sw::value<sw::ZKC_VW_BIG>(0), vws_env = (uint32_t)sw::value<sw::ZKC_VW_SMALL>(0);
        const uint32_t vws = nb <= 4 ? 64u : vws_env ? vws_env : nb < 32 ? 256u : 2048u, vwb = nb <= 4 ? 256u : vwb_env ? vwb_env : nb < 32 ? 1024u : 4096u;
        size_t lone_entries = 0; for (int q = 0; q < nb; q++) lone_entries += (size_t)msm_nw(MSM_C_G2_LONE) * (listed ? vms[q].nB : nv);
        const size_t deep_wires = (size_t)sw::value<sw::ZKC_DEEP_WIRES>(16000);
        size_t live_wires = 0; for (int q = 0; q < nb; q++) live_wires += listed ? (size_t)vms[q].nA + vms[q].nB + vms[q].nC : 2 * (size_t)nv + nc;
        const bool deep = zk->c_deep != 0 && nb > 2 && live_wires >= 3 * deep_wires * (size_t)nb;
        const int cw = deep ? zk->c_deep : zk->c_sec;
        const uint32_t oA = deep ? zk->offA_deep : zk->offA, oB1 = deep ? zk->offB1_deep : zk->offB1, oC = deep ? zk->offC_deep : zk->offC;
        const int c2 = (nb <= 2 && zk->d_g2_29_lone && lone_entries <= LN.w2.max_entries) ? MSM_C_G2_LONE : cw;
        const uint32_t vwg2_env = (uint32_t)sw::value<sw::ZKC_VW_G2>(0);
        j1.clear(vws, vwb, MSM_MAX_VW_G1); j2.clear(c2 == MSM_C_G2_LONE ? 128u : (vwg2_env && nb >= 32) ? vwg2_env : vws, 1024, MSM_MAX_VW_PER_JOB);
        for (int q = 0; q < nb; q++) j1.add(LN.d_p + 8 * (size_t)n * q, nullptr, n, zk->offH, n, 0, zk->c_h);
        size_t tree_entries = 0; for (int q = 0; q < nb; q++) tree_entries += (size_t)msm_nw(zk->c_h) * n + (size_t)msm_nw(zk->c_sec) * (listed ? 2 * (size_t)vms[q].nA + 2 * (size_t)vms[q].nB + vms[q].nC : 4 * (size_t)nv + nc);
        const bool tree = zk->d_fb4 != nullptr && nb <= 2 && 6 * nb <= LN.w1.max_jobs && tree_entries <= LN.w1.max_entries && (size_t)nb * (5 * msm_half(zk->c_sec) + msm_half(zk->c_h)) <= LN.w1.max_buckets;
        BlindArgs ba{}; ba.rs = CS.d_rs + 64 * (size_t)p0; ba.nv = nv;
        for (int q = 0; q < nb; q++) {
            const uint32_t* w = w0 + (size_t)q * nv * 8;
            uint32_t* bs = tree ? LN.d_bs + (size_t)q * 2 * nv * 8 : nullptr;
            if (tree) { ba.w[q] = w; ba.out[q] = bs; }
            if (listed) {
                const zkc_zkey::Fold::VMap& vm = vms[q];
                j1.add(w, vm.d + vm.offA, vm.nA, oA, nv, 0, cw);
                j1.add(w, vm.d + vm.offB, vm.nB, oB1, nv, 0, cw);
                j1.add(w, vm.d + vm.offC, vm.nC, oC, nc, (int32_t)np + 1, cw);
                if (tree) { j1.add(bs, vm.d + vm.offA, vm.nA, oA, nv, 0, cw); j1.add(bs + 8ull * nv, vm.d + vm.offB, vm.nB, oB1, nv, 0, cw); }
                j2.add(w, vm.d + vm.offB, vm.nB, 0, nv, 0, c2);
                if (tree) { ba.mapA[q] = vm.d + vm.offA; ba.nA[q] = vm.nA; ba.mapB[q] = vm.d + vm.offB; ba.nB[q] = vm.nB; }
            } else {
                j1.add(w, nullptr, nv, oA, nv, 0, cw);
                j1.add(w, nullptr, nv, oB1, nv, 0, cw);
                j1.add(w + 8ull * (np + 1), nullptr, nc, oC, nc, 0, cw);
                if (tree) { j1.add(bs, nullptr, nv, oA, nv, 0, cw); j1.add(bs + 8ull * nv, nullptr, nv, oB1, nv, 0, cw); }
                j2.add(w, nullptr, nv, 0, nv, 0, c2);
                if (tree) { ba.mapA[q] = ba.mapB[q] = nullptr; ba.nA[q] = ba.nB[q] = nv; }
            }
        }
        if (tree && (rc = blind_scalars_launch(ctx, st, ba, nb))) return rc;
        FinalizeArgs fa{};
        fa.r1 = (const G1XYZZ*)LN.w1.results + (size_t)slot * LN.w1.max_jobs; fa.r2 = (const G2XYZZ*)LN.w2.results + (size_t)slot * LN.w2.max_jobs;
        fa.foldA = zk->fold.d_foldA; fa.foldB1 = zk->fold.d_foldB1; fa.foldC = zk->fold.d_foldC; fa.foldB2 = zk->fold.d_foldB2; fa.fold_n = can_fold ? L.n : 0;
        for (int q = 0; q < nb; q++) { fa.dc[q] = fold ? dcq[q] : (uint8_t)255; fa.ds[q] = fold ? dsq[q] : (uint8_t)255; }
        fa.tblDelta1 = zk->d_tblDelta1; fa.tblAlpha1 = zk->d_tblAlpha1; fa.tblBeta1 = zk->d_tblBeta1; fa.tblDelta2 = zk->d_tblDelta2;
        fa.alpha1 = zk->alpha1; fa.beta2 = zk->beta2; fa.rs = CS.d_rs + 64 * (size_t)p0; fa.out = CS.d_proofs + 256 * (size_t)p0; fa.scratch = LN.d_fin;
        fa.per = tree ? 5 : 3; fa.fb4 = zk->d_fb4; fa.fb4g2 = zk->d_fb4g2; fa.out_xyzz = CS.d_xyzz + 512 * (size_t)p0;
        const bool g2_early = !sw::on<sw::ZKC_G2_LATE>();
        const bool g2_hold_env = sw::on<sw::ZKC_G2_ACC_HOLD>(), g2_early_env = sw::on<sw::ZKC_G2_ACC_EARLY>();
        const bool g2_acc_with_sort = g2_hold_env || ((nb < 32 || !one_lane) && !g2_early_env);
        if (g2_early) {
            if ((rc = msm_pass_g2(zk, LN.w2, j2, slot, false, st2, g2_acc_with_sort ? LN.ev_ntt : nullptr))) return rc;
            if (tree && (rc = finalize_tree_g2_launch(ctx, st2, fa, nb))) return rc;
            ZKC_HIP_CHECK(ctx, hipEventRecord(LN.ev_msm2, st2));
        }
        tr[3] = now_ms();
        ZKC_HIP_CHECK(ctx, hipStreamWaitEvent(st, LN.ev_red, 0));
        const bool red_split = sw::on<sw::ZKC_REDUCE_STREAM>() && !zk->serial_streams && nb >= 32;
        if ((rc = msm_pass_g1(zk, LN.w1, j1, slot, false, st, LN.ev_sorted, LN.ev_acc, (red_split && LS.red) ? LS.red : nullptr, LN.ev_red))) return rc;
        tr[4] = now_ms();
        if (!g2_early) {
            ZKC_HIP_CHECK(ctx, hipStreamWaitEvent(st2, LN.ev_sorted, 0));
            if ((rc = msm_pass_g2(zk, LN.w2, j2, slot, false, st2))) return rc;
            if (tree && (rc = finalize_tree_g2_launch(ctx, st2, fa, nb))) return rc;
            ZKC_HIP_CHECK(ctx, hipEventRecord(LN.ev_msm2, st2));
        }
        if (want_publics)
            ZKC_HIP_CHECK(ctx, hipMemcpy2DAsync(h_pub + 32ull * np * p0, 32ull * np, w0 + 8, 32ull * nv, 32ull * np, nb, hipMemcpyDeviceToHost, st));
        ZKC_HIP_CHECK(ctx, hipEventRecord(LN.ev_msm, st));
        if (mv_prefetch && p0 + per_pass < B) {
            const int p1 = p0 + per_pass, nb1 = std::min(per_pass, B - p1);
            ZKC_HIP_CHECK(ctx, hipStreamWaitEvent(fin, sw::on<sw::ZKC_MV_PREFETCH_AT_NTT>() ? LN.ev_ntt : LN.ev_sorted, 0));
            ZKC_HIP_CHECK(ctx, hipStreamWaitEvent(fin, CS.ev_chunk[pass + 1], 0));
            if ((rc = h_matvec_dev(zk, LN, (const uint32_t*)d_wtns + (size_t)p1 * nv * 8, nb1, fin))) return rc;
            ZKC_HIP_CHECK(ctx, hipEventRecord(LN.ev_mv, fin));
        }
        hipStream_t bl = ((tree || lane0 >= 0) && npasses == 1) ? st : fin;
        if (bl == fin) { ZKC_HIP_CHECK(ctx, hipStreamWaitEvent(fin, LN.ev_msm, 0)); ZKC_HIP_CHECK(ctx, hipStreamWaitEvent(fin, LN.ev_red, 0)); }
        else { if (LN.npass >= 2) ZKC_HIP_CHECK(ctx, hipStreamWaitEvent(st, LN.ev_fin[slot ^ 1], 0)); if (red_split) ZKC_HIP_CHECK(ctx, hipStreamWaitEvent(st, LN.ev_red, 0)); }
        if (!tree) ZKC_HIP_CHECK(ctx, hipStreamWaitEvent(bl, LN.ev_msm2, 0));
        if ((rc = finalize_launch(ctx, bl, fa, nb))) return rc;
        if (tree) ZKC_HIP_CHECK(ctx, hipStreamWaitEvent(bl, LN.ev_msm2, 0));
        if (tree) { ZKC_HIP_CHECK(ctx, hipMemcpyAsync(CS.h_xyzz + 512ull * p0, CS.d_xyzz + 512 * (size_t)p0, 512ull * nb, hipMemcpyDeviceToHost, bl)); for (int q = 0; q < nb; q++) CS.as_xyzz[p0 + q] = 1; }
        else ZKC_HIP_CHECK(ctx, hipMemcpyAsync(CS.h_out + 256ull * p0, CS.d_proofs + 256 * (size_t)p0, 256ull * nb, hipMemcpyDeviceToHost, bl));
        ZKC_HIP_CHECK(ctx, hipEventRecord(LN.ev_fin[slot], bl));
        if (bl == st) done_on_st_lane = li;
        tr[5] = now_ms();
        if (trace_host) fprintf(stderr, "[zkc host] pass %2d: start %8.2f | chunk wait %6.2f | h_evals %6.2f | g2 pass %6.2f | g1 pass %6.2f | blinding %6.2f ms\n", pass, tr[0] - t_begin,
                                tr[1] - tr[0], tr[2] - tr[1], tr[3] - tr[2], tr[4] - tr[3], tr[5] - tr[4]);
    }
    for (int l = 0; l < zk->nlanes; l++) if (CS.lanes_used >> l & 1) { const LaneSt ls = lane_st(zk, ctx->lanes[l]); ZKC_HIP_CHECK(ctx, hipEventRecord(CS.ev_done[l], done_on_st_lane == l ? ls.st : ls.fin)); }
    CS.B = B; CS.pending = true;
    return ZKC_OK;
}
static std::atomic<unsigned long long> g_early_retries{0};
extern "C" unsigned long long zkc_debug_early_retries(void) { return g_early_retries.load(); }
int zkc::prove_batch_finish(zkc_zkey* zk, int cs, uint8_t* proofs, uint8_t* publics) {
    if (!zk || !proofs || cs < 0 || cs >= CALL_SLOTS) return zkc_fail(zk ? zk->ctx : nullptr, ZKC_ERR_BAD_ARG, "prove_batch_finish: bad argument");
    zkc_zkey::CallSlot& CS = zk->call[cs];
    if (!CS.pending) return zkc_fail(zk->ctx, ZKC_ERR_BAD_ARG, "prove_batch_finish: no call in flight on this slot");
    hipError_t e = hipSuccess;
    for (int l = 0; l < zk->nlanes && e == hipSuccess; l++) if (CS.lanes_used >> l & 1) e = zkc_wait_event(CS.ev_done[l], CS.B <= 2 ? 6000u : 0u);
    CS.pending = false;
    if (e != hipSuccess) { ZKC_LOCK(zk->ctx); return zkc_fail(zk->ctx, ZKC_ERR_HIP, std::string("prove_batch_finish: ") + hipGetErrorString(e)); }
    if (CS.early_n) {
        const WitnessLayout L = WitnessLayout::make(zk->nLevels);
        for (int q = 0; q < CS.early_n; q++) {
            if ((int32_t)CS.h_early[q] != ZKC_W_OK) continue;
            for (int t = 0; t < 2; t++) {
                const uint32_t* f = CS.h_early + CS.early_cap + ((size_t)q * 2 + t) * L.n;
                int D = 0; for (int g = 0; g < L.n - 1; g++) if (f[g]) D = g + 1;
                if (f[L.n - 1] || D > (int)CS.early_depth[2 * q + t]) {
                    if (!CS.arg_inputs) { g_early_retries++; int rc = prove_batch_begin(zk, cs, CS.arg_wtns, CS.arg_nw, CS.B, CS.h_rs_copy.data(), CS.arg_publics, nullptr, nullptr, CS.arg_lane0, nullptr, nullptr, true); if (rc) return rc; return prove_batch_finish(zk, cs, proofs, publics); }
                    ZKC_LOCK(zk->ctx); return zkc_fail(zk->ctx, ZKC_ERR_GENERIC, "prove_batch_finish: the witness does not fold at the depth its inputs gave (internal error)");
                }
            }
        }
    }
    memcpy(proofs, CS.h_out, 256ull * CS.B);
    for (int q = 0; q < CS.B; q++) if (CS.as_xyzz[q]) {
        const uint8_t* x = CS.h_xyzz + 512 * (size_t)q; uint8_t* o = proofs + 256 * (size_t)q;
// ... 52 lines not shown
```

### zk-franchise-proof-circuit_amd/csrc/zkc_prover.h

```cpp
#pragma once
#include <cstring>
#include "zkc_internal.h"
#include "zkc_curve.h"

namespace zkc {
constexpr int MSM_C_BIG = 17, MSM_C_SMALL = 12;
constexpr int MSM_C_G2_LONE = 8;
inline long long first_unreduced_wire(const void* w, size_t count) {
    const uint8_t* p = (const uint8_t*)w;
    for (size_t i = 0; i < count; i++) {
        uint32_t t[8]; memcpy(t, p + 32 * i, 32);
        if (t[7] >= FrParams::p[7] && !fp_std_lt_p<FrParams>(t)) return (long long)i;
    }
    return -1;
}
inline std::string unreduced_wire_msg(long long wire) { return "Witness value at wire " + std::to_string(wire) + " is not below the field order r"; }
inline int msm_c_for(size_t W) { return W < 12000 ? 12 : W < 22000 ? 13 : W < 90000 ? 15 : W < 180000 ? 16 : 17; }
constexpr int msm_nw(int c) { return (254 + c) / c; }
constexpr int msm_half(int c) { return 1 << (c - 1); }
constexpr int MSM_VW_MIN = 64, MSM_MAX_VW_PER_JOB = 64;
constexpr int MSM_MAX_VW_G1 = 256;
constexpr int MSM_SEG_MIN = 16;
#ifndef ZKC_MSM_SEG
#define ZKC_MSM_SEG 128
#endif
constexpr int MSM_SEG = ZKC_MSM_SEG;
constexpr int MSM_MERGE_T = 8;
constexpr int MSM_MAX_HEAVY = 1 << 20;
constexpr int MSM_MAX_JOBS = 512;
constexpr int MAX_LANES = 4, CALL_SLOTS = 4;
static_assert(sw::rows[sw::ZKC_C_SECTIONS].hi == MSM_C_BIG && sw::rows[sw::ZKC_C_H].hi == MSM_C_BIG && sw::rows[sw::ZKC_C_DEEP].hi == MSM_C_BIG, "zkc_switches.h: MSM_C_BIG");
static_assert(sw::rows[sw::ZKC_INFLIGHT].hi == MSM_MAX_JOBS / 4 && sw::rows[sw::ZKC_SERVICE_PASS].hi == MSM_MAX_JOBS / 4, "zkc_switches.h: MSM_MAX_JOBS / 4");
static_assert(sw::rows[sw::ZKC_LANES].hi == MAX_LANES && sw::rows[sw::ZKC_SERVICE_WORKERS].hi == MAX_LANES, "zkc_switches.h: MAX_LANES");

struct MsmJob {
    const uint32_t* scalars;
    const uint32_t* vmap;
    uint32_t count;
    uint32_t tbl_off;
    uint32_t tbl_count;
    int32_t pt_shift;
    uint32_t c, nw, vw;
    uint32_t ent_off, win_off;
    uint32_t bucket0, bin0, hbits, lbits, tile0, cnt0;
};
struct FinalizeArgs {
    const G1XYZZ* r1; const G2XYZZ* r2;
    const G1XYZZ *foldA, *foldB1, *foldC; const G2XYZZ* foldB2; int fold_n;
    uint8_t dc[MSM_MAX_JOBS / 4], ds[MSM_MAX_JOBS / 4];
    const G1Affine *tblDelta1, *tblAlpha1, *tblBeta1; const G2Affine* tblDelta2;
    G1Affine alpha1; G2Affine beta2;
    const uint8_t* rs; uint8_t* out;
    void* scratch;
    int per; const G1XYZZ* fb4; const G2XYZZ* fb4g2;
    uint8_t* out_xyzz;
};
constexpr int FB4_WIN = 64, FB4_ROW = 15;
struct BlindArgs { const uint32_t* w[2]; const uint32_t* mapA[2]; const uint32_t* mapB[2]; uint32_t nA[2], nB[2]; uint32_t* out[2]; const uint8_t* rs; uint32_t nv; };
constexpr int MSM_TILE = 256, MSM_TILE_SCALARS = 1024;
constexpr uint32_t MSM_MAX_HBITS = 10;
struct MsmJobList {
    MsmJob job[MSM_MAX_JOBS]; int njobs; uint32_t total_buckets, total_entries, total_windows, total_bins, total_tiles, total_tilecnt;
    uint32_t hs, hb, nbig;
    uint32_t hbits_big, hbits_small;
    uint32_t vw_big = 1024;
    uint32_t vw_small = 256;
    void add(const uint32_t* scalars, const uint32_t* vmap, uint32_t count, uint32_t tbl_off, uint32_t tbl_count, int32_t pt_shift, int c) {
        MsmJob& j = job[njobs++];
        uint32_t vw = c >= 16 ? vw_big : vw_small;
        if (vw > (uint32_t)msm_half(c)) vw = (uint32_t)msm_half(c);
        while ((uint32_t)msm_half(c) / vw > max_vw_per_job) vw <<= 1;
        j = MsmJob{scalars, vmap, count, tbl_off, tbl_count, pt_shift, (uint32_t)c, (uint32_t)msm_nw(c), vw, total_entries, total_windows, 0, 0, 0, 0, 0, 0};
        total_entries += count * (uint32_t)msm_nw(c); total_windows += (uint32_t)msm_half(c) / vw;
    }
    uint32_t max_vw_per_job = 256;
    void clear(uint32_t vw_small_jobs = 256, uint32_t vw_big_jobs = 1024, uint32_t max_per_job = 256) { vw_small = vw_small_jobs; vw_big = vw_big_jobs; max_vw_per_job = max_per_job; njobs = 0; total_buckets = total_entries = total_windows = total_bins = total_tiles = total_tilecnt = 0; hs = hb = nbig = 0; }
    bool finish() {
        hs = 0xffffffffu; hb = 0;
        for (int j = 0; j < njobs; j++) { const uint32_t h = 1u << (job[j].c - 1); hs = h < hs ? h : hs; hb = h > hb ? h : hb; }
        nbig = 0; total_buckets = total_bins = total_tiles = total_tilecnt = 0; hbits_big = hbits_small = 0;
        for (int j = 0; j < njobs; j++) {
            MsmJob& q = job[j]; const uint32_t h = 1u << (q.c - 1);
            if (h != hs && h != hb) return false;
            if (h == hb) { if ((uint32_t)j != nbig) return false; nbig++; }
            uint32_t hbits = q.c - 1 < 8 ? q.c - 1 : 8, lbits = q.c - 1 - hbits;
            const uint64_t rows = (uint64_t)q.nw * q.tbl_count;
            while (lbits > 8 || (lbits > 0 && rows >= (1ull << (31 - lbits)))) { lbits--; hbits++; }
            if (hbits > MSM_MAX_HBITS || rows >= (1ull << (31 - lbits))) return false;
            q.hbits = hbits; q.lbits = lbits;
            { uint32_t& cls = h == hb ? hbits_big : hbits_small; cls = (cls == 0 || cls == hbits) ? hbits : 0xffu; }
            q.bucket0 = total_buckets; total_buckets += h;
            q.bin0 = total_bins; total_bins += 1u << hbits;
            const uint32_t nt = (q.count + MSM_TILE_SCALARS - 1) / MSM_TILE_SCALARS;
            q.tile0 = total_tiles; total_tiles += nt; q.cnt0 = total_tilecnt; total_tilecnt += nt << hbits;
        }
        return true;
    }
    ZKC_HD uint32_t id_of(uint32_t d, uint32_t j) const { return job[j].bucket0 + d; }
    ZKC_HD uint32_t job_of_bin(uint32_t bin) const {
        if (hbits_big != 0xffu && hbits_small != 0xffu) {
            const uint32_t lim = nbig << hbits_big;
            return bin < lim ? bin >> hbits_big : nbig + ((bin - lim) >> hbits_small);
        }
        uint32_t lo = 0, hi = (uint32_t)njobs - 1;
        while (lo < hi) { const uint32_t mid = (lo + hi + 1) >> 1; if (job[mid].bin0 <= bin) lo = mid; else hi = mid - 1; }
        return lo;
    }
    ZKC_HD void decode(uint32_t id, uint32_t& d, uint32_t& j) const {
        const uint32_t lim = hb * nbig;
        if (id < lim) { j = id / hb; d = id - j * hb; }
        else { const uint32_t t = id - lim, q = t / hs; j = nbig + q; d = t - q * hs; }
    }
};
struct MsmWindow { uint32_t bucket0, out, per; };

struct MsmWork {
    uint32_t *vals = nullptr, *vals2 = nullptr;
    uint32_t *hist = nullptr, *bin_start = nullptr;
    uint32_t *tilecnt = nullptr; size_t max_tilecnt = 0;
    uint32_t *off = nullptr, *bcnt = nullptr;
    uint32_t *segcnt = nullptr, *segoff = nullptr, *seg2bucket = nullptr, *heavy = nullptr;
    uint32_t *seglen = nullptr, *perm = nullptr;
    uint32_t *scan_blk = nullptr, *lencnt = nullptr; size_t max_lencnt = 0;
    void *partial = nullptr;
    void *wres = nullptr;
    void *results = nullptr;
    void *h_results = nullptr;
    MsmJobList* d_jobs = nullptr;
    MsmWindow* d_windows = nullptr; size_t max_buckets = 0, max_bins = 0, max_windows = 0;
    uint16_t* d_tilejob = nullptr; uint16_t* h_tilejob[2] = {nullptr, nullptr}; size_t max_tiles = 0;
    MsmJobList* h_jobs[2] = {nullptr, nullptr}; MsmWindow* h_windows[2] = {nullptr, nullptr}; hipEvent_t h_ev[2] = {nullptr, nullptr}; int h_next = 0;
    size_t max_entries = 0, max_segments = 0; int max_jobs = 0; size_t xyzz_size = 0;
};
}

struct zkc_lane {
    hipStream_t st = nullptr, st2 = nullptr, fin = nullptr;
    hipStream_t red = nullptr; hipEvent_t ev_red = nullptr;
    zkc::Fr *d_abc = nullptr, *d_t = nullptr; uint32_t* d_p = nullptr;
    void* d_fin = nullptr;
    uint32_t* d_bs = nullptr;
    zkc::MsmWork w1, w2;
    size_t cap_abc = 0, cap_p = 0, cap_fin = 0, cap_bs = 0, bytes = 0; bool made = false;
    hipEvent_t ev_msm = nullptr, ev_msm2 = nullptr, ev_sorted = nullptr, ev_ntt = nullptr, ev_mv = nullptr, ev_acc = nullptr, ev_fin[2] = {nullptr, nullptr}; int npass = 0;
};

struct zkc_zkey {
    zkc_ctx* ctx = nullptr;
    uint32_t nVars = 0, nPub = 0, n = 0, logn = 0, nCoeffs = 0;
    int nLevels = -1;
    zkc::G1Affine alpha1, beta1, delta1;
    zkc::G2Affine beta2, gamma2, delta2;
    std::vector<zkc::G1Affine> ic;
    uint32_t *d_perm = nullptr, *d_rowlen = nullptr, *d_jdptr = nullptr, *d_col = nullptr; zkc::Fr* d_val = nullptr; uint32_t nlong = 0;
    uint32_t n_unit_coeffs = 0;
    zkc::Fr *d_tw_fwd = nullptr, *d_tw_inv = nullptr, *d_coset = nullptr;
    zkc::Fr *d_coset_br = nullptr;
    uint32_t *d_tw_fwd29 = nullptr, *d_tw_inv29 = nullptr;
    zkc::G1Affine* d_g1 = nullptr; zkc::G2Affine* d_g2 = nullptr;
    uint32_t* d_g2_29 = nullptr;
    uint32_t* d_g2_29_lone = nullptr;
    uint32_t offA = 0, offB1 = 0, offC = 0, offH = 0;
    int c_deep = 0; uint32_t offA_deep = 0, offB1_deep = 0, offC_deep = 0; uint32_t* d_g2_29_deep = nullptr;
    int c_h = zkc::MSM_C_BIG;
    int c_sec = zkc::MSM_C_SMALL;
    int max_inflight = 0;
    uint8_t sha256[32] = {0};
    size_t bytes_tables = 0;
    uint8_t fingerprint[32] = {0};
    int nlanes = 1; bool serial_streams = false;
    zkc::G1Affine *d_tblDelta1 = nullptr, *d_tblAlpha1 = nullptr, *d_tblBeta1 = nullptr; zkc::G2Affine* d_tblDelta2 = nullptr;
    uint32_t *d_depths = nullptr, *h_depths = nullptr; size_t depths_cap = 0;
    zkc::G1XYZZ* d_fb4 = nullptr; zkc::G2XYZZ* d_fb4g2 = nullptr; int fb4_bases = 0;
    struct CallSlot {
        uint8_t *d_rs = nullptr, *d_proofs = nullptr; size_t cap = 0;
        uint8_t* h_out = nullptr;
        uint8_t* h_rs = nullptr;
        uint8_t *d_xyzz = nullptr, *h_xyzz = nullptr; std::vector<uint8_t> as_xyzz;
        hipEvent_t ev_done[zkc::MAX_LANES] = {};
        std::vector<hipEvent_t> ev_chunk;
        uint32_t lanes_used = 0;
        int B = 0; bool pending = false;
        uint32_t *d_flags = nullptr, *h_flags = nullptr; size_t flags_cap = 0;
        int32_t* d_status3 = nullptr; size_t status3_cap = 0;
        int early_n = 0; std::vector<uint8_t> early_depth; uint32_t* h_early = nullptr; size_t early_cap = 0;
        const void* arg_wtns = nullptr; uint32_t arg_nw = 0; bool arg_publics = false, arg_inputs = false; int arg_lane0 = -1; hipEvent_t arg_wait = nullptr; std::vector<uint8_t> h_rs_copy;
    } call[zkc::CALL_SLOTS];
    struct Fold {
        std::vector<zkc::G1XYZZ> baseA, baseB1, baseC; std::vector<zkc::G2XYZZ> baseB2;
        std::vector<zkc::G1XYZZ> sufA[2], sufB1[2], sufC[2]; std::vector<zkc::G2XYZZ> sufB2[2];
        struct VMap { uint32_t* d = nullptr; uint32_t offA = 0, nA = 0, offB = 0, nB = 0, offC = 0, nC = 0; };
        std::map<std::pair<int, int>, VMap> vmaps;
        std::vector<uint8_t> infA, infB, infC;
        zkc::G1XYZZ *d_foldA = nullptr, *d_foldB1 = nullptr, *d_foldC = nullptr; zkc::G2XYZZ* d_foldB2 = nullptr;
        bool ready = false;
    } fold;
};

namespace zkc {
int ntt_run(zkc_ctx* ctx, hipStream_t st, const Fr* src, Fr* dst, const uint32_t* tw29, const Fr* scale, int logn, int nvec);
int ntt_make_tw29(zkc_ctx* ctx, const Fr* d_tw, uint32_t count, uint32_t** out);
struct TwiddleTables { Fr *fwd = nullptr, *inv = nullptr; uint32_t *fwd29 = nullptr, *inv29 = nullptr; };
int ntt_twiddle_tables(zkc_ctx* ctx, int logn, bool keep_fr, TwiddleTables* out);
int msm_g2_window_table29(zkc_ctx* ctx, const G2Affine* d_bases, uint32_t count, int c, const char* what, uint32_t** out);
int msm_g2_rows29(zkc_ctx* ctx, const G2Affine* d_points, size_t n, const char* what, uint32_t** out);
int ntt_pair_run(zkc_ctx* ctx, hipStream_t st, Fr* data, const uint32_t* tw_inv29, const uint32_t* tw_fwd29, const Fr* scale_br, int logn, int nvec);
int ntt_bitrev_table(zkc_ctx* ctx, const Fr* d_src, Fr** out, int logn);
int msm_work_alloc(zkc_ctx* ctx, MsmWork& w, size_t max_entries, size_t max_buckets, int max_jobs, bool g2);
void msm_work_free(MsmWork& w);
int msm_pass_g1(zkc_zkey* zk, MsmWork& w, const MsmJobList& jl, int slot, bool to_host, hipStream_t st, hipEvent_t ev_sorted = nullptr, hipEvent_t ev_acc = nullptr,
                hipStream_t st_red = nullptr, hipEvent_t ev_red = nullptr);
int msm_pass_g2(zkc_zkey* zk, MsmWork& w, const MsmJobList& jl, int slot, bool to_host, hipStream_t st, hipEvent_t wait_before_acc = nullptr);
int msm_bucket_entries(zkc_ctx* ctx, MsmWork& w, const MsmJobList& jl, hipStream_t st, unsigned long long* d_entry_counter = nullptr);
int msm_build_segments(zkc_ctx* ctx, MsmWork& w, const MsmJobList& jl, uint32_t seg, size_t seg_bound, hipStream_t st);
int finalize_launch(zkc_ctx* ctx, hipStream_t st, const FinalizeArgs& a, int nproofs);
int finalize_tree_g2_launch(zkc_ctx* ctx, hipStream_t st, const FinalizeArgs& a, int nproofs);
int fb4_build(zkc_ctx* ctx, hipStream_t st, const G1XYZZ* d_bases, int nbases, G1XYZZ* d_out, const G2XYZZ& delta2, const G2XYZZ& beta2, const G2XYZZ& beta2_base, G2XYZZ* d_out2);
int blind_scalars_launch(zkc_ctx* ctx, hipStream_t st, const BlindArgs& a, int nproofs);
int prove_batch_begin(zkc_zkey* zk, int cs, const void* d_wtns, uint32_t nWitness, int B, const uint8_t* rs, bool want_publics, const void* d_inputs, int32_t* d_status,
                      int lane0 = -1, hipEvent_t wait_first = nullptr, const uint8_t* host_depths = nullptr, bool no_early = false);
int prove_batch_finish(zkc_zkey* zk, int cs, uint8_t* proofs, uint8_t* publics);
int prove_reserve(zkc_zkey* zk, int inflight);
int zkey_load_opts(zkc_ctx* ctx, const void* zkey_bytes, size_t len, int nlanes, int max_inflight, zkc_zkey** out);
size_t zkey_device_bytes(const zkc_zkey* zk, size_t* tables, size_t* work);
size_t finalize_scratch_bytes(int nproofs);
int msm_precompute_g1(zkc_ctx* ctx, uint32_t count, G1Affine* d_table, int c);
int msm_precompute_g2(zkc_ctx* ctx, uint32_t count, G2Affine* d_table, int c);
int msm_g2_table29(zkc_ctx* ctx, const G2Affine* d_table, uint32_t* d_out, size_t count);
int fold_group_sums_g1(zkc_ctx* ctx, const G1Affine* tbl, const uint32_t* d_scalars, const uint32_t* d_wires, uint32_t nw, int32_t pt_shift,
                       const uint32_t* d_gstart, uint32_t ngroups, G1XYZZ* h_out);
int fold_group_sums_g1_ws(zkc_ctx* ctx, const G1Affine* tbl, const uint32_t* d_scalars, const uint32_t* d_wires, uint32_t nw, const uint32_t* d_gstart, uint32_t ngroups,
                          G1XYZZ* d_tmp , G1XYZZ* d_out , G1XYZZ* h_out);
int fold_group_sums_g2(zkc_ctx* ctx, const G2Affine* tbl, const uint32_t* d_scalars, const uint32_t* d_wires, uint32_t nw, int32_t pt_shift,
                       const uint32_t* d_gstart, uint32_t ngroups, G2XYZZ* h_out);
}
```

### zk-franchise-proof-circuit_amd/csrc/zkc_switches.h

```cpp
#pragma once
#include <climits>
#include <cstdlib>
#include <optional>

namespace zkc { namespace sw {

enum Kind { SET, OFF_IF_ZERO, ON_IF_ONE, NUMBER, NUMBER_LONG, NUMBER_U64, TEXT };
enum When { PROCESS, LIVE };
constexpr long long ANY = LLONG_MIN;

#define ZKC_SWITCHES(X)                                                                                                                                                   \
                                                                                                                                            \
    X(ZKC_DEVICE,               TEXT,        ANY, ANY,   LIVE,    "service creation: the GPUs of the default proving service: \"2\", \"0,1,2,3\", \"all\"; unset: every visible device") \
    X(ZKC_INFLIGHT,             NUMBER,      1,   128,   LIVE,    "key load: proofs per pipeline pass (census key 64, any other 96, fewer for a large circuit); at most MSM_MAX_JOBS / 4") \
    X(ZKC_LANES,                NUMBER,      1,   4,     LIVE,    "key load: pipeline lanes the passes of a batch call rotate over (census key MAX_LANES = 4, any other 1)")      \
    X(ZKC_DEEP_TABLES,          NUMBER,      ANY, ANY,   LIVE,    "key load: 0 leaves out the second section tables that passes of deep voters take, 2 builds them for a census key of any size (default 1)") \
    X(ZKC_G2_LONE_TABLE,        OFF_IF_ZERO, ANY, ANY,   LIVE,    "key load: =0 skips the 8-bit-window G2 table of the lone-proof path")                                          \
    X(ZKC_BLIND_TREE,           OFF_IF_ZERO, ANY, ANY,   LIVE,    "key load: =0 gives a key whose passes of one or two proofs take the general blinding kernels")                 \
    X(ZKC_SERVICE_WORKERS,      NUMBER,      1,   4,     LIVE,    "service creation: workers (= lanes of a service key) per GPU (4); at most MAX_LANES")                          \
    X(ZKC_SERVICE_PASS,         NUMBER,      1,   128,   LIVE,    "service creation: proofs per pass of a service key (64); at most MSM_MAX_JOBS / 4")                            \
    X(ZKC_SERVICE_KEYS,         NUMBER,      1,   64,    LIVE,    "service creation: keys kept resident per GPU (4)")                                                             \
    X(ZKC_SERVICE_MAX_BATCH,    NUMBER,      1,   4096,  LIVE,    "service creation: requests one worker takes per call (256)")                                                   \
    X(ZKC_SERVICE_MIN_BATCH,    NUMBER,      1,   ANY,   LIVE,    "service creation: requests a collecting worker waits for before it goes (16)")                                 \
    X(ZKC_SERVICE_SPILL,        NUMBER,      1,   ANY,   LIVE,    "service creation: queue length at which a cold GPU is brought up (32)")                                        \
    X(ZKC_SERVICE_BUSY_WAIT_US, NUMBER,      0,   ANY,   LIVE,    "service creation: microseconds a collecting worker waits for more requests (300)")                             \
    X(ZKC_SERVICE_RESERVE,      OFF_IF_ZERO, ANY, ANY,   PROCESS, "=0: a service key load does not reserve a full pass of work space on every lane; the lanes grow on demand")    \
    X(ZKC_DEVICE_BLOCKING_SYNC, ON_IF_ONE,   ANY, ANY,   LIVE,    "context creation: =1 asks HIP for blocking waits on the device (hipDeviceScheduleBlockingSync)")               \
    X(ZKC_SPIN_WAIT,            SET,         ANY, ANY,   PROCESS, "set (any value, 0 included): host waits use hipEventSynchronize instead of polling with short sleeps")         \
    X(ZKC_VERIFY_BATCH_GPU,     NUMBER,      ANY, ANY,   LIVE,    "per verify call: 0 keeps the Miller loops of zkc_verify_batch on the host, positive forces the GPU, negative or unset: GPU from 128 proofs") \
    X(ZKC_NO_SHA_NI,            SET,         ANY, ANY,   PROCESS, "set (any value, 0 included): portable SHA-256 instead of the CPU's SHA extensions")                            \
                                                                                                                              \
    X(ZKC_NO_FOLD,              SET,         ANY, ANY,   LIVE,    "key load: set (any value, 0 included): no constant folding of the voter-independent witness part for this key") \
    X(ZKC_SERIAL_STREAMS,       SET,         ANY, ANY,   LIVE,    "key load: set (any value, 0 included): every stage of this key's passes on the context's one stream (isolated stage times)") \
    X(ZKC_C_SECTIONS,           NUMBER,      8,   17,    LIVE,    "key load: window bits of the witness sections (census key 12, any other by its wire count); at most MSM_C_BIG") \
    X(ZKC_C_H,                  NUMBER,      8,   17,    LIVE,    "key load: window bits of the H section (census key 17, any other by its domain size); at most MSM_C_BIG")      \
    X(ZKC_C_DEEP,               NUMBER,      13,  17,    LIVE,    "key load: window bits of the second section tables (by the wire count); at most MSM_C_BIG")                    \
    X(ZKC_DEEP_WIRES,           NUMBER_LONG, ANY, ANY,   PROCESS, "live wires per section and proof from which a pass takes the second section tables (16000)")                   \
    X(ZKC_WITNESS_GROUP,        NUMBER,      1,   ANY,   PROCESS, "passes whose voters share one witness launch in a batch call (8)")                                             \
    X(ZKC_VW_BIG,               NUMBER,      ANY, ANY,   PROCESS, "buckets per reduction wave of the H jobs in passes of more than four proofs (0 or unset: 4096, 1024 below 32 proofs)") \
    X(ZKC_VW_SMALL,             NUMBER,      ANY, ANY,   PROCESS, "the same for the witness sections (0 or unset: 2048, 256 below 32 proofs)")                                    \
    X(ZKC_VW_G2,                NUMBER,      ANY, ANY,   PROCESS, "the same for the G2 jobs of passes of 32 proofs and more (0 or unset: as the witness sections)")              \
    X(ZKC_G2_ACC,               NUMBER,      ANY, ANY,   PROCESS, "form of the G2 accumulation: 0 registers hold the next row, 1 / 2 LDS-DMA prefetch at one / two waves per SIMD (0)") \
    X(ZKC_G2_BUCKET_WAVE,       OFF_IF_ZERO, ANY, ANY,   PROCESS, "=0: small G2 passes keep lane-per-segment accumulation instead of half a wave per bucket")                     \
    X(ZKC_G2_LATE,              SET,         ANY, ANY,   PROCESS, "set (any value, 0 included): the G2 MSM of a pass starts after the G1 sort instead of with the pass")          \
    X(ZKC_G2_ACC_HOLD,          SET,         ANY, ANY,   PROCESS, "set (any value, 0 included): the G2 accumulation always waits for the G1 stream to leave its transforms")      \
    X(ZKC_G2_ACC_EARLY,         SET,         ANY, ANY,   PROCESS, "set (any value, 0 included): the G2 accumulation never waits for them (ZKC_G2_ACC_HOLD wins)")                 \
    X(ZKC_ACC_CHAIN,            OFF_IF_ZERO, ANY, ANY,   PROCESS, "=0: the G1 accumulations of a context's lanes are not chained one behind the other")                           \
    X(ZKC_REDUCE_STREAM,        ON_IF_ONE,   ANY, ANY,   PROCESS, "=1: the bucket reduction of a full pass runs on a stream of its own (the lanes then get that stream)")         \
    X(ZKC_MATVEC_UNITS,         OFF_IF_ZERO, ANY, ANY,   PROCESS, "=0: buildABC multiplies by its +-1 coefficients instead of adding the wire")                                   \
    X(ZKC_MATVEC_INLINE,        SET,         ANY, ANY,   PROCESS, "set (any value, 0 included): buildABC of the next pass is not prefetched on the blinding stream")              \
    X(ZKC_MV_PREFETCH_AT_NTT,   ON_IF_ONE,   ANY, ANY,   PROCESS, "=1: that prefetch starts beside the pass' bucketing instead of beside its accumulation")                       \
    X(ZKC_EARLY_LAYOUT,         OFF_IF_ZERO, ANY, ANY,   PROCESS, "=0: one-pass calls of more than two voters wait for their fold flags instead of reading the depths off the inputs") \
    X(ZKC_NOFOLD_LISTS,         OFF_IF_ZERO, ANY, ANY,   PROCESS, "=0: unfolded passes keep the wires whose bases are at infinity")                                               \
    X(ZKC_NTT_SEPARATE,         SET,         ANY, ANY,   PROCESS, "set (any value, 0 included): two self-contained transforms instead of the fused pair")                         \
    X(ZKC_NTT_RADIX,            NUMBER,      ANY, ANY,   PROCESS, "below 4: the head transform kernel runs one stage at a time instead of two (4)")                               \
    X(ZKC_FINALIZE_WAVES,       SET,         ANY, ANY,   PROCESS, "set (any value, 0 included): the one-wave-per-task blinding kernel for every pass")                            \
    X(ZKC_VERIFY_CHUNK,         NUMBER,      2,   16384, LIVE,    "per verify call: pairs per round of Miller-loop kernels (16384)")                                              \
    X(ZKC_SMT_WAVE_MAX,         NUMBER_U64,  ANY, ANY,   LIVE,    "per check call: census proof batches up to this size take the wave-per-proof form (64; 0: never)")            \
    X(ZKC_TRACE_HOST,           SET,         ANY, ANY,   PROCESS, "set (any value, 0 included): prints where the enqueueing thread spends its time, per pass")                    \
    X(ZKC_VERIFY_TRACE,         SET,         ANY, ANY,   LIVE,    "per verify call: set (any value, 0 included): prints the stage times of zkc_verify_batch")                     \
    X(ZKC_DEBUG_SYNC,           SET,         ANY, ANY,   PROCESS, "set (any value, 0 included): synchronises after and logs every MSM launch; read when the library is loaded")   \
                                                                                                                                                \
    X(ZKC_TEST_FAIL_ALLOC,      NUMBER,      ANY, ANY,   LIVE,    "lane growth: the work-space allocation for this many proofs in flight or more fails")                          \
    X(ZKC_TEST_FAIL_KEY_LOADS,  NUMBER,      ANY, ANY,   LIVE,    "service key load: fails as out of memory while the device holds this many keys or more")

enum Id {
#define X(name, kind, lo, hi, when, doc) name,
    ZKC_SWITCHES(X)
#undef X
    COUNT
};
struct Row { const char* name; Kind kind; long long lo, hi; When when; const char* doc; };
inline constexpr Row rows[COUNT] = {
#define X(name, kind, lo, hi, when, doc) {#name, kind, lo, (hi) == ANY ? LLONG_MAX : (hi), when, doc},
    ZKC_SWITCHES(X)
#undef X
};

struct Raw { bool set; long long num; const char* str; };
inline Raw read(const Row& r) {
    const char* e = getenv(r.name);
    if (!e) return {false, 0, nullptr};
    const long long v = r.kind == NUMBER_U64 ? (long long)strtoull(e, nullptr, 10) : r.kind == NUMBER_LONG ? (long long)atol(e) : (long long)atoi(e);
    return {true, v < r.lo ? r.lo : v > r.hi ? r.hi : v, e};
}
template <Id I> inline Raw get() {
    if constexpr (rows[I].when == PROCESS) { static const Raw cached = read(rows[I]); return cached; }
    else return read(rows[I]);
}
constexpr bool is_number(Kind k) { return k == NUMBER || k == NUMBER_LONG || k == NUMBER_U64; }

template <Id I> inline bool on() {
    static_assert(rows[I].kind == SET || rows[I].kind == OFF_IF_ZERO || rows[I].kind == ON_IF_ONE, "not an on/off switch");
    const Raw r = get<I>();
    return rows[I].kind == SET ? r.set : rows[I].kind == OFF_IF_ZERO ? !(r.set && r.num == 0) : (r.set && r.num == 1);
}
template <Id I> inline std::optional<long long> given() {
    static_assert(is_number(rows[I].kind), "not a number");
    const Raw r = get<I>();
    return r.set ? std::optional<long long>(r.num) : std::nullopt;
}
template <Id I> inline long long value(long long dflt) { return given<I>().value_or(dflt); }
template <Id I> inline const char* text() {
    static_assert(rows[I].kind == TEXT && rows[I].when == LIVE, "not a live text switch");
    return get<I>().str;
}

}}
```

Baseline: 3111.

## Merge the C-section MSM into the H MSM job using a shared wide-window table

At key load, the C-section bases are appended behind the H bases and precomputed with H's window width. In passes of 32 or more proofs, each proof's C scalars are then summed inside its H job instead of in a separate MSM job. Result slots are remapped and the C slot is zeroed. This removes one job per proof and its bucket setup and reduction overhead, at the cost of a larger H table and more entries on the wider window. It also adds per-kind entry counters for profiling.

```diff
diff --git a/include/zkcensus.h b/include/zkcensus.h
--- a/include/zkcensus.h
+++ b/include/zkcensus.h
@@ -170,6 +170,7 @@
 
 int zkc_profile_enable(zkc_ctx* ctx, uint32_t mask);
 int zkc_profile_read(zkc_ctx* ctx, int category, double* total_ms, uint64_t* launches, uint64_t* alg_bytes);
+int zkc_profile_madds(zkc_ctx* ctx, uint64_t out[6]);
 
 int zkc_setup_from_r1cs(const char* r1cs_path, uint64_t seed, const char* zkey_path, const char* vkey_json_path,
                         char* err, size_t errlen);
diff --git a/zk-franchise-proof-circuit_amd/_native.py b/zk-franchise-proof-circuit_amd/_native.py
--- a/zk-franchise-proof-circuit_amd/_native.py
+++ b/zk-franchise-proof-circuit_amd/_native.py
@@ -88,6 +88,7 @@
     L.zkc_msm_g1_dev.argtypes = [vp, vp, ctypes.c_char_p]
     L.zkc_msm_g1_free.argtypes = [vp]; L.zkc_msm_g1_free.restype = None
     L.zkc_profile_read.argtypes = [vp, ctypes.c_int, ctypes.POINTER(ctypes.c_double), ctypes.POINTER(ctypes.c_uint64), ctypes.POINTER(ctypes.c_uint64)]
+    L.zkc_profile_madds.argtypes = [vp, ctypes.POINTER(ctypes.c_uint64)]
     L.zkc_setup_from_r1cs.argtypes = [ctypes.c_char_p, ctypes.c_uint64, ctypes.c_char_p, ctypes.c_char_p, ctypes.c_char_p, ctypes.c_size_t]
     L.zkc_setup_from_r1cs_dev.argtypes = [vp, ctypes.c_char_p, ctypes.c_uint64, ctypes.c_char_p, ctypes.c_char_p, ctypes.c_char_p, ctypes.c_size_t]
     L.zkc_setup_stats.argtypes = [ctypes.POINTER(ctypes.c_double)]
diff --git a/zk-franchise-proof-circuit_amd/csrc/zkc_api.hip b/zk-franchise-proof-circuit_amd/csrc/zkc_api.hip
--- a/zk-franchise-proof-circuit_amd/csrc/zkc_api.hip
+++ b/zk-franchise-proof-circuit_amd/csrc/zkc_api.hip
@@ -71,8 +71,8 @@
     for (auto& r : ctx->prof.pending) { ctx->prof.free_events.push_back(r.a); ctx->prof.free_events.push_back(r.b); }
     ctx->prof.pending.clear();
     for (int i = 0; i < ZKC_PROF_NCAT; i++) { ctx->prof.ms[i] = 0; ctx->prof.launches[i] = 0; ctx->prof.bytes[i] = 0; }
-    if (!ctx->d_prof_entries && hipMalloc((void**)&ctx->d_prof_entries, 8) != hipSuccess) ctx->d_prof_entries = nullptr;
-    if (ctx->d_prof_entries) (void)hipMemset(ctx->d_prof_entries, 0, 8);
+    if (!ctx->d_prof_entries && hipMalloc((void**)&ctx->d_prof_entries, 8 * (1 + ZKC_PROF_MADD_KINDS)) != hipSuccess) ctx->d_prof_entries = nullptr;
+    if (ctx->d_prof_entries) (void)hipMemset(ctx->d_prof_entries, 0, 8 * (1 + ZKC_PROF_MADD_KINDS));
     ctx->prof.mask = mask;
     return ZKC_OK;
 }
@@ -90,6 +90,18 @@
         unsigned long long v = 0; (void)hipMemcpyAsync(&v, ctx->d_prof_entries, 8, hipMemcpyDeviceToHost, ctx->stream); (void)hipStreamSynchronize(ctx->stream); ctx->prof.launches[cat] = v;
     }
     if (total_ms) *total_ms = ctx->prof.ms[cat]; if (launches) *launches = ctx->prof.launches[cat]; if (alg_bytes) *alg_bytes = ctx->prof.bytes[cat];
+    return ZKC_OK;
+}
+extern "C" int zkc_profile_madds(zkc_ctx* ctx, uint64_t out[6]) {
+    if (!ctx || !out) return ZKC_ERR_BAD_ARG;
+    ZKC_LOCK(ctx);
+    ZKC_HIP_CHECK(ctx, hipSetDevice(ctx->device));
+    if (!ctx->d_prof_entries) return zkc_fail(ctx, ZKC_ERR_BAD_ARG, "zkc_profile_madds: profiling has not been enabled on this context");
+    static_assert(ZKC_PROF_MADD_KINDS == 6, "include/zkcensus.h: zkc_profile_madds");
+    unsigned long long v[1 + ZKC_PROF_MADD_KINDS] = {0};
+    ZKC_HIP_CHECK(ctx, hipDeviceSynchronize());
+    ZKC_HIP_CHECK(ctx, hipMemcpy(v, ctx->d_prof_entries, sizeof(v), hipMemcpyDeviceToHost));
+    for (int k = 0; k < ZKC_PROF_MADD_KINDS; k++) out[k] = v[1 + k];
     return ZKC_OK;
 }
 
diff --git a/zk-franchise-proof-circuit_amd/csrc/zkc_internal.h b/zk-franchise-proof-circuit_amd/csrc/zkc_internal.h
--- a/zk-franchise-proof-circuit_amd/csrc/zkc_internal.h
+++ b/zk-franchise-proof-circuit_amd/csrc/zkc_internal.h
@@ -15,6 +15,7 @@
 
 enum { ZKC_PROF_WITNESS = 0, ZKC_PROF_MATVEC = 1, ZKC_PROF_NTT = 2, ZKC_PROF_MSM_SORT = 3, ZKC_PROF_MSM_ACC_G1 = 4, ZKC_PROF_MSM_ACC_G2 = 5,
        ZKC_PROF_MSM_REDUCE = 6, ZKC_PROF_MSM_G1_STREAMED = 7 , ZKC_PROF_NCAT = 8 };
+constexpr int ZKC_PROF_MADD_KINDS = 6;
 struct zkc_prof {
     uint32_t mask = 0;
     struct Rec { hipEvent_t a, b; int cat; };
diff --git a/zk-franchise-proof-circuit_amd/csrc/zkc_msm.hip b/zk-franchise-proof-circuit_amd/csrc/zkc_msm.hip
--- a/zk-franchise-proof-circuit_amd/csrc/zkc_msm.hip
+++ b/zk-franchise-proof-circuit_amd/csrc/zkc_msm.hip
@@ -407,7 +407,7 @@
         if ((int)threadIdx.x < st) { Acc29 t = sh[threadIdx.x]; f29_pt_add(t, t, sh[threadIdx.x + st]); sh[threadIdx.x] = t; }
         __syncthreads();
     }
-    if (threadIdx.x == 0) results[j] = f29_pt_is_inf(sh[0]) ? XYZZ<Fq>::inf() : f29_pt_to_xyzz(sh[0]);
+    if (threadIdx.x == 0) results[jl->job[j].out] = f29_pt_is_inf(sh[0]) ? XYZZ<Fq>::inf() : f29_pt_to_xyzz(sh[0]);
 }
 
 __global__ void __launch_bounds__(MSM_MAX_VW_PER_JOB)
@@ -439,7 +439,7 @@
         if ((int)threadIdx.x < st) { Acc29G2 t = sh[threadIdx.x]; f29g2_pt_add(t, t, sh[threadIdx.x + st]); sh[threadIdx.x] = t; }
         __syncthreads();
     }
-    if (threadIdx.x == 0) results[j] = f29g2_pt_is_inf(sh[0]) ? XYZZ<Fq2>::inf() : f29g2_pt_to_xyzz(sh[0]);
+    if (threadIdx.x == 0) results[jl->job[j].out] = f29g2_pt_is_inf(sh[0]) ? XYZZ<Fq2>::inf() : f29g2_pt_to_xyzz(sh[0]);
 }
 
 template <class F>
diff --git a/zk-franchise-proof-circuit_amd/csrc/zkc_msm_sort.hip b/zk-franchise-proof-circuit_amd/csrc/zkc_msm_sort.hip
--- a/zk-franchise-proof-circuit_amd/csrc/zkc_msm_sort.hip
+++ b/zk-franchise-proof-circuit_amd/csrc/zkc_msm_sort.hip
@@ -12,10 +12,11 @@
 #pragma unroll
         for (int q = 0; q < 8; q++) t.s[k][q] = 0;
         if (t.live[k]) {
-            const uint32_t wire = job.vmap ? job.vmap[i] : i;
-            const uint4* sp = reinterpret_cast<const uint4*>(job.scalars + 8 * (size_t)wire); const uint4 a = sp[0], b = sp[1];
+            const bool hd = i < job.split; const uint32_t r = i - job.split;
+            const uint32_t wire = hd ? i : job.vmap ? job.vmap[r] : r;
+            const uint4* sp = reinterpret_cast<const uint4*>((hd ? job.head : job.scalars) + 8 * (size_t)wire); const uint4 a = sp[0], b = sp[1];
             t.s[k][0] = a.x; t.s[k][1] = a.y; t.s[k][2] = a.z; t.s[k][3] = a.w; t.s[k][4] = b.x; t.s[k][5] = b.y; t.s[k][6] = b.z; t.s[k][7] = b.w;
-            t.pt[k] = (uint32_t)((int32_t)wire - job.pt_shift);
+            t.pt[k] = hd ? i : job.split + (uint32_t)((int32_t)wire - job.pt_shift);
         }
     }
 }
@@ -73,7 +74,10 @@
         __syncthreads();
     }
     const uint32_t end = carry_sh;
-    if (entry_counter && threadIdx.x == 0) atomicAdd(entry_counter, (unsigned long long)(end - job.ent_off));
+    if (entry_counter && threadIdx.x == 0) {
+        atomicAdd(entry_counter, (unsigned long long)(end - job.ent_off));
+        atomicAdd(entry_counter + 1 + (job.kind < (uint32_t)MSM_KINDS ? job.kind : 0u), (unsigned long long)(end - job.ent_off));
+    }
     for (uint32_t b = threadIdx.x; b < nbins; b += 256) {
         const uint32_t st = c[b * ntiles], en = b + 1 < nbins ? c[(b + 1) * ntiles] : end;
         bin_start[job.bin0 + b] = st; hist[job.bin0 + b] = en - st;
diff --git a/zk-franchise-proof-circuit_amd/csrc/zkc_prove.hip b/zk-franchise-proof-circuit_amd/csrc/zkc_prove.hip
--- a/zk-franchise-proof-circuit_amd/csrc/zkc_prove.hip
+++ b/zk-franchise-proof-circuit_amd/csrc/zkc_prove.hip
@@ -235,19 +235,27 @@
     { const int dt = (int)sw::value<sw::ZKC_DEEP_TABLES>(1); const auto e_c = sw::given<sw::ZKC_C_DEEP>();
       const int cd = e_c ? (int)*e_c : msm_c_for(dt == 2 ? (size_t)40000 : (size_t)nv * 4 / 5);
       zk->c_deep = (zk->nLevels >= 0 && (nv >= (1u << 16) || dt == 2) && zk->c_sec < cd && dt != 0) ? cd : 0; }
+    const bool h_wide_enough = zk->c_h >= std::max(zk->c_sec, zk->c_deep);
     zk->c_h = std::max(zk->c_h, std::max(zk->c_sec, zk->c_deep));
     const int NWB = msm_nw(zk->c_h);
+    {
+        uint32_t hb0, lb0, hb1, lb1;
+        const bool fits = MsmJobList::level1((uint32_t)zk->c_h, (uint64_t)NWB * n, hb0, lb0) && MsmJobList::level1((uint32_t)zk->c_h, (uint64_t)NWB * ((uint64_t)n + nc), hb1, lb1) && hb0 == hb1;
+        zk->c_in_h = sw::value<sw::ZKC_C_IN_H>(1) != 0 && nc > 0 && h_wide_enough && fits;
+        zk->h_rows = zk->c_in_h ? n + nc : n;
+    }
     zk->offA = 0; zk->offB1 = NWS * nv; zk->offC = 2 * NWS * nv; zk->offH = 2 * NWS * nv + NWS * nc;
     const int NWD = zk->c_deep ? msm_nw(zk->c_deep) : 0;
-    zk->offA_deep = zk->offH + NWB * n; zk->offB1_deep = zk->offA_deep + NWD * nv; zk->offC_deep = zk->offB1_deep + NWD * nv;
-    const size_t g1_points = (size_t)NWS * (2 * (size_t)nv + nc) + (size_t)NWB * n + (size_t)NWD * (2 * (size_t)nv + nc);
+    zk->offA_deep = zk->offH + NWB * zk->h_rows; zk->offB1_deep = zk->offA_deep + NWD * nv; zk->offC_deep = zk->offB1_deep + NWD * nv;
+    const size_t g1_points = (size_t)NWS * (2 * (size_t)nv + nc) + (size_t)NWB * zk->h_rows + (size_t)NWD * (2 * (size_t)nv + nc);
     if (g1_points >= (1ull << 31)) return bail(zkc_fail(ctx, ZKC_ERR_FORMAT, "zkey too large for 31-bit point indices"));
     if ((rc = dmalloc(ctx, &zk->d_g1, g1_points)) || (rc = dmalloc(ctx, &zk->d_g2, (size_t)NWS * nv))) return bail(rc);
     ZKC_UP(zk->d_g1 + zk->offA, sec[5], 64ull * nv); ZKC_UP(zk->d_g1 + zk->offB1, sec[6], 64ull * nv);
     ZKC_UP(zk->d_g1 + zk->offC, sec[8], 64ull * nc); ZKC_UP(zk->d_g1 + zk->offH, sec[9], 64ull * n);
+    if (zk->c_in_h) ZKC_UP(zk->d_g1 + zk->offH + n, sec[8], 64ull * nc);
     ZKC_UP(zk->d_g2, sec[7], 128ull * nv);
     if ((rc = msm_precompute_g1(ctx, nv, zk->d_g1 + zk->offA, zk->c_sec)) || (rc = msm_precompute_g1(ctx, nv, zk->d_g1 + zk->offB1, zk->c_sec)) ||
-        (rc = msm_precompute_g1(ctx, nc, zk->d_g1 + zk->offC, zk->c_sec)) || (rc = msm_precompute_g1(ctx, n, zk->d_g1 + zk->offH, zk->c_h)) ||
+        (rc = msm_precompute_g1(ctx, nc, zk->d_g1 + zk->offC, zk->c_sec)) || (rc = msm_precompute_g1(ctx, zk->h_rows, zk->d_g1 + zk->offH, zk->c_h)) ||
         (rc = msm_precompute_g2(ctx, nv, zk->d_g2, zk->c_sec))) return bail(rc);
     if ((rc = dmalloc(ctx, &zk->d_g2_29, 60 * (size_t)NWS * nv)) || (rc = msm_g2_table29(ctx, zk->d_g2, zk->d_g2_29, (size_t)NWS * nv))) return bail(rc);
     if (zk->c_deep) {
@@ -460,17 +468,20 @@
 }
 
 extern "C" int zkc_msm_debug(zkc_zkey* zk, int which, const void* d_scalars, uint32_t count, void* host_out) {
-    if (!zk || !d_scalars || !host_out || which < 0 || which > 4) return ZKC_ERR_BAD_ARG;
+    if (!zk || !d_scalars || !host_out || which < 0 || which > 5) return ZKC_ERR_BAD_ARG;
     zkc_ctx* ctx = zk->ctx;
     ZKC_LOCK(ctx);
     ZKC_HIP_CHECK(ctx, hipSetDevice(ctx->device)); ZKC_HIP_CHECK(ctx, hipStreamSynchronize(ctx->stream));
     { int rc0 = lanes_ensure(zk, 1, 0, 1); if (rc0) return rc0; }
     zkc_lane& L0 = ctx->lanes[0]; const hipStream_t st_l0 = lane_st(zk, L0).st;
-    const uint32_t full = which == 3 ? zk->nVars - zk->nPub - 1 : which == 4 ? zk->n : zk->nVars;
+    const uint32_t nc = zk->nVars - zk->nPub - 1;
+    const uint32_t full = which == 3 ? nc : which == 4 ? zk->n : which == 5 ? zk->n + nc : zk->nVars;
+    if (which == 5 && !zk->c_in_h) return zkc_fail(ctx, ZKC_ERR_BAD_ARG, "zkc_msm_debug: this key has no C table behind its H table (ZKC_C_IN_H)");
     if (count != full) return zkc_fail(ctx, ZKC_ERR_BAD_ARG, "zkc_msm_debug: count must equal the section size");
     static thread_local MsmJobList jl; jl.clear(256, 1024, which == 2 ? (uint32_t)MSM_MAX_VW_PER_JOB : (uint32_t)MSM_MAX_VW_G1);
     const uint32_t offs[5] = {zk->offA, zk->offB1, 0, zk->offC, zk->offH};
-    jl.add((const uint32_t*)d_scalars, nullptr, count, offs[which], full, 0, which == 4 ? zk->c_h : zk->c_sec);
+    if (which == 5) jl.add_head((const uint32_t*)d_scalars, zk->n, (const uint32_t*)d_scalars + 8 * (size_t)zk->n, nullptr, nc, zk->offH, zk->h_rows, 0, zk->c_h, MSM_KIND_HC);
+    else jl.add((const uint32_t*)d_scalars, nullptr, count, offs[which], which == 4 ? zk->h_rows : full, 0, which == 4 ? zk->c_h : zk->c_sec);
     int rc = which == 2 ? msm_pass_g2(zk, L0.w2, jl, 0, true, st_l0) : msm_pass_g1(zk, L0.w1, jl, 0, true, st_l0); if (rc) return rc;
     ZKC_HIP_CHECK(ctx, hipStreamSynchronize(st_l0));
     if (which == 2) wr_g2_std((uint8_t*)host_out, xyzz_to_affine(*(G2XYZZ*)L0.w2.h_results));
@@ -624,7 +635,14 @@
         const int c2 = (nb <= 2 && zk->d_g2_29_lone && lone_entries <= LN.w2.max_entries) ? MSM_C_G2_LONE : cw;
         const uint32_t vwg2_env = (uint32_t)sw::value<sw::ZKC_VW_G2>(0);
         j1.clear(vws, vwb, MSM_MAX_VW_G1); j2.clear(c2 == MSM_C_G2_LONE ? 128u : (vwg2_env && nb >= 32) ? vwg2_env : vws, 1024, MSM_MAX_VW_PER_JOB);
-        for (int q = 0; q < nb; q++) j1.add(LN.d_p + 8 * (size_t)n * q, nullptr, n, zk->offH, n, 0, zk->c_h);
+        const int cih = (int)sw::value<sw::ZKC_C_IN_H>(1);
+        const bool merged = zk->c_in_h && nb > 2 && (cih == 2 || (cih == 1 && nb >= 32));
+        for (int q = 0; q < nb; q++) {
+            const uint32_t* hq = LN.d_p + 8 * (size_t)n * q; const uint32_t* w = w0 + (size_t)q * nv * 8;
+            if (!merged) j1.add(hq, nullptr, n, zk->offH, zk->h_rows, 0, zk->c_h, MSM_KIND_H);
+            else if (listed) j1.add_head(hq, n, w, vms[q].d + vms[q].offC, vms[q].nC, zk->offH, zk->h_rows, (int32_t)np + 1, zk->c_h, MSM_KIND_HC);
+            else j1.add_head(hq, n, w + 8ull * (np + 1), nullptr, nc, zk->offH, zk->h_rows, 0, zk->c_h, MSM_KIND_HC);
+        }
         size_t tree_entries = 0; for (int q = 0; q < nb; q++) tree_entries += (size_t)msm_nw(zk->c_h) * n + (size_t)msm_nw(zk->c_sec) * (listed ? 2 * (size_t)vms[q].nA + 2 * (size_t)vms[q].nB + vms[q].nC : 4 * (size_t)nv + nc);
         const bool tree = zk->d_fb4 != nullptr && nb <= 2 && 6 * nb <= LN.w1.max_jobs && tree_entries <= LN.w1.max_entries && (size_t)nb * (5 * msm_half(zk->c_sec) + msm_half(zk->c_h)) <= LN.w1.max_buckets;
         BlindArgs ba{}; ba.rs = CS.d_rs + 64 * (size_t)p0; ba.nv = nv;
@@ -634,20 +652,26 @@
             if (tree) { ba.w[q] = w; ba.out[q] = bs; }
             if (listed) {
                 const zkc_zkey::Fold::VMap& vm = vms[q];
-                j1.add(w, vm.d + vm.offA, vm.nA, oA, nv, 0, cw);
-                j1.add(w, vm.d + vm.offB, vm.nB, oB1, nv, 0, cw);
-                j1.add(w, vm.d + vm.offC, vm.nC, oC, nc, (int32_t)np + 1, cw);
+                j1.add(w, vm.d + vm.offA, vm.nA, oA, nv, 0, cw, MSM_KIND_A);
+                j1.add(w, vm.d + vm.offB, vm.nB, oB1, nv, 0, cw, MSM_KIND_B1);
+                if (!merged) j1.add(w, vm.d + vm.offC, vm.nC, oC, nc, (int32_t)np + 1, cw, MSM_KIND_C);
                 if (tree) { j1.add(bs, vm.d + vm.offA, vm.nA, oA, nv, 0, cw); j1.add(bs + 8ull * nv, vm.d + vm.offB, vm.nB, oB1, nv, 0, cw); }
                 j2.add(w, vm.d + vm.offB, vm.nB, 0, nv, 0, c2);
                 if (tree) { ba.mapA[q] = vm.d + vm.offA; ba.nA[q] = vm.nA; ba.mapB[q] = vm.d + vm.offB; ba.nB[q] = vm.nB; }
             } else {
-                j1.add(w, nullptr, nv, oA, nv, 0, cw);
-                j1.add(w, nullptr, nv, oB1, nv, 0, cw);
-                j1.add(w + 8ull * (np + 1), nullptr, nc, oC, nc, 0, cw);
+                j1.add(w, nullptr, nv, oA, nv, 0, cw, MSM_KIND_A);
+                j1.add(w, nullptr, nv, oB1, nv, 0, cw, MSM_KIND_B1);
+                if (!merged) j1.add(w + 8ull * (np + 1), nullptr, nc, oC, nc, 0, cw, MSM_KIND_C);
                 if (tree) { j1.add(bs, nullptr, nv, oA, nv, 0, cw); j1.add(bs + 8ull * nv, nullptr, nv, oB1, nv, 0, cw); }
                 j2.add(w, nullptr, nv, 0, nv, 0, c2);
                 if (tree) { ba.mapA[q] = ba.mapB[q] = nullptr; ba.nA[q] = ba.nB[q] = nv; }
             }
+        }
+        if (merged) {
+            for (int q = 0; q < nb; q++) for (int k = 0; k < 2; k++) j1.job[nb + 2 * q + k].out = (uint32_t)(nb + 3 * q + k);
+            G1XYZZ* res = (G1XYZZ*)LN.w1.results + (size_t)slot * LN.w1.max_jobs;
+            if (4 * nb > LN.w1.max_jobs) return zkc_fail(ctx, ZKC_ERR_BAD_ARG, "prove_batch_begin: result slots of a merged pass");
+            ZKC_HIP_CHECK(ctx, hipMemset2DAsync(res + nb + 2, 3 * sizeof(G1XYZZ), 0, sizeof(G1XYZZ), (size_t)nb, st));
         }
         if (tree && (rc = blind_scalars_launch(ctx, st, ba, nb))) return rc;
         FinalizeArgs fa{};
diff --git a/zk-franchise-proof-circuit_amd/csrc/zkc_prover.h b/zk-franchise-proof-circuit_amd/csrc/zkc_prover.h
--- a/zk-franchise-proof-circuit_amd/csrc/zkc_prover.h
+++ b/zk-franchise-proof-circuit_amd/csrc/zkc_prover.h
@@ -43,7 +43,12 @@
     uint32_t c, nw, vw;
     uint32_t ent_off, win_off;
     uint32_t bucket0, bin0, hbits, lbits, tile0, cnt0;
-};
+    const uint32_t* head; uint32_t split;
+    uint32_t out;
+    uint32_t kind;
+};
+enum { MSM_KIND_OTHER = 0, MSM_KIND_A = 1, MSM_KIND_B1 = 2, MSM_KIND_C = 3, MSM_KIND_H = 4, MSM_KIND_HC = 5, MSM_KINDS = 6 };
+static_assert(MSM_KINDS == ZKC_PROF_MADD_KINDS, "zkc_internal.h: ZKC_PROF_MADD_KINDS");
 struct FinalizeArgs {
     const G1XYZZ* r1; const G2XYZZ* r2;
     const G1XYZZ *foldA, *foldB1, *foldC; const G2XYZZ* foldB2; int fold_n;
@@ -65,16 +70,25 @@
     uint32_t hbits_big, hbits_small;
     uint32_t vw_big = 1024;
     uint32_t vw_small = 256;
-    void add(const uint32_t* scalars, const uint32_t* vmap, uint32_t count, uint32_t tbl_off, uint32_t tbl_count, int32_t pt_shift, int c) {
+    void add(const uint32_t* scalars, const uint32_t* vmap, uint32_t count, uint32_t tbl_off, uint32_t tbl_count, int32_t pt_shift, int c, uint32_t kind = MSM_KIND_OTHER) {
         MsmJob& j = job[njobs++];
         uint32_t vw = c >= 16 ? vw_big : vw_small;
         if (vw > (uint32_t)msm_half(c)) vw = (uint32_t)msm_half(c);
         while ((uint32_t)msm_half(c) / vw > max_vw_per_job) vw <<= 1;
-        j = MsmJob{scalars, vmap, count, tbl_off, tbl_count, pt_shift, (uint32_t)c, (uint32_t)msm_nw(c), vw, total_entries, total_windows, 0, 0, 0, 0, 0, 0};
+        j = MsmJob{scalars, vmap, count, tbl_off, tbl_count, pt_shift, (uint32_t)c, (uint32_t)msm_nw(c), vw, total_entries, total_windows, 0, 0, 0, 0, 0, 0, nullptr, 0, (uint32_t)njobs - 1, kind};
         total_entries += count * (uint32_t)msm_nw(c); total_windows += (uint32_t)msm_half(c) / vw;
+    }
+    void add_head(const uint32_t* head, uint32_t split, const uint32_t* scalars, const uint32_t* vmap, uint32_t count, uint32_t tbl_off, uint32_t tbl_count, int32_t pt_shift, int c, uint32_t kind) {
+        add(scalars, vmap, split + count, tbl_off, tbl_count, pt_shift, c, kind);
+        job[njobs - 1].head = head; job[njobs - 1].split = split;
     }
     uint32_t max_vw_per_job = 256;
     void clear(uint32_t vw_small_jobs = 256, uint32_t vw_big_jobs = 1024, uint32_t max_per_job = 256) { vw_small = vw_small_jobs; vw_big = vw_big_jobs; max_vw_per_job = max_per_job; njobs = 0; total_buckets = total_entries = total_windows = total_bins = total_tiles = total_tilecnt = 0; hs = hb = nbig = 0; }
+    static bool level1(uint32_t c, uint64_t rows, uint32_t& hbits, uint32_t& lbits) {
+        hbits = c - 1 < 8 ? c - 1 : 8; lbits = c - 1 - hbits;
+        while (lbits > 8 || (lbits > 0 && rows >= (1ull << (31 - lbits)))) { lbits--; hbits++; }
+        return hbits <= MSM_MAX_HBITS && rows < (1ull << (31 - lbits));
+    }
     bool finish() {
         hs = 0xffffffffu; hb = 0;
         for (int j = 0; j < njobs; j++) { const uint32_t h = 1u << (job[j].c - 1); hs = h < hs ? h : hs; hb = h > hb ? h : hb; }
@@ -83,10 +97,8 @@
             MsmJob& q = job[j]; const uint32_t h = 1u << (q.c - 1);
             if (h != hs && h != hb) return false;
             if (h == hb) { if ((uint32_t)j != nbig) return false; nbig++; }
-            uint32_t hbits = q.c - 1 < 8 ? q.c - 1 : 8, lbits = q.c - 1 - hbits;
-            const uint64_t rows = (uint64_t)q.nw * q.tbl_count;
-            while (lbits > 8 || (lbits > 0 && rows >= (1ull << (31 - lbits)))) { lbits--; hbits++; }
-            if (hbits > MSM_MAX_HBITS || rows >= (1ull << (31 - lbits))) return false;
+            uint32_t hbits, lbits;
+            if (!level1(q.c, (uint64_t)q.nw * q.tbl_count, hbits, lbits)) return false;
             q.hbits = hbits; q.lbits = lbits;
             { uint32_t& cls = h == hb ? hbits_big : hbits_small; cls = (cls == 0 || cls == hbits) ? hbits : 0xffu; }
             q.bucket0 = total_buckets; total_buckets += h;
@@ -162,6 +174,7 @@
     uint32_t* d_g2_29_lone = nullptr;
     uint32_t offA = 0, offB1 = 0, offC = 0, offH = 0;
     int c_deep = 0; uint32_t offA_deep = 0, offB1_deep = 0, offC_deep = 0; uint32_t* d_g2_29_deep = nullptr;
+    uint32_t h_rows = 0; bool c_in_h = false;
     int c_h = zkc::MSM_C_BIG;
     int c_sec = zkc::MSM_C_SMALL;
     int max_inflight = 0;
diff --git a/zk-franchise-proof-circuit_amd/csrc/zkc_switches.h b/zk-franchise-proof-circuit_amd/csrc/zkc_switches.h
--- a/zk-franchise-proof-circuit_amd/csrc/zkc_switches.h
+++ b/zk-franchise-proof-circuit_amd/csrc/zkc_switches.h
@@ -35,6 +35,7 @@
     X(ZKC_C_SECTIONS,           NUMBER,      8,   17,    LIVE,    "key load: window bits of the witness sections (census key 12, any other by its wire count); at most MSM_C_BIG") \
     X(ZKC_C_H,                  NUMBER,      8,   17,    LIVE,    "key load: window bits of the H section (census key 17, any other by its domain size); at most MSM_C_BIG")      \
     X(ZKC_C_DEEP,               NUMBER,      13,  17,    LIVE,    "key load: window bits of the second section tables (by the wire count); at most MSM_C_BIG")                    \
+    X(ZKC_C_IN_H,               NUMBER,      0,   2,     LIVE,    "key load and per pass: 0 keeps the C section a job of its own (and builds no second C table), 1 sums it inside the H job in passes of 32 proofs and more, 2 in every pass of more than two proofs (1)") \
     X(ZKC_DEEP_WIRES,           NUMBER_LONG, ANY, ANY,   PROCESS, "live wires per section and proof from which a pass takes the second section tables (16000)")                   \
     X(ZKC_WITNESS_GROUP,        NUMBER,      1,   ANY,   PROCESS, "passes whose voters share one witness launch in a batch call (8)")                                             \
     X(ZKC_VW_BIG,               NUMBER,      ANY, ANY,   PROCESS, "buckets per reduction wave of the H jobs in passes of more than four proofs (0 or unset: 4096, 1024 below 32 proofs)") \
```

New measurement: 3138, median of 6. No clear change (+0.9%).
